# ducha-aiki/mods

Measured on AMD Instinct MI355X. Metric: image-pairs/sec (1024x768, HessAff+RootSIFT over the affine view ladder, MFMA FGINN match, LO-RANSAC H), higher is better.
Workload: dtype f32 (detect/describe) + u8 on the int8 matrix cores (distance matrix)

## Files before the change

include/modsx.h:

```cpp
#ifndef MODSX_H
#define MODSX_H
#include <stdint.h>
#ifdef __cplusplus
extern "C" {
#endif

#define MODSX_VERSION 100

typedef enum modsx_status {
  MODSX_OK = 0,
  MODSX_ERR_ARG = -1,
  MODSX_ERR_DEVICE = -2,
  MODSX_ERR_NOMEM = -3,
  MODSX_ERR_INTERNAL = -4,
  MODSX_ERR_CAPACITY = -5,
  MODSX_ERR_TIMEOUT = -6
} modsx_status;

enum { MODSX_FIXED_TH = 0, MODSX_RELATIVE_TH = 1, MODSX_FIXED_REG_NUMBER = 2, MODSX_RELATIVE_REG_NUMBER = 3,
       MODSX_NOT_LESS_THAN_REGIONS = 4 };
enum { MODSX_DET_HESSIAN = 0, MODSX_DET_DOG = 1, MODSX_DET_HARRIS = 2, MODSX_DET_MSER = 3 };
enum { MODSX_DESC_SIFT = 0, MODSX_DESC_ROOT_SIFT = 1, MODSX_DESC_HALF_SIFT = 2, MODSX_DESC_HALF_ROOT_SIFT = 3 };
#define MODSX_MAX_DESC 4
enum { MODSX_HESSIAN_DARK = 0, MODSX_HESSIAN_BRIGHT = 1, MODSX_HESSIAN_SADDLE = 2 };
// ... 118 lines not shown
int modsx_resize_half(modsx_ctx *ctx, const modsx_image *img, float *out, int *orows, int *ocols);

int modsx_response(modsx_ctx *ctx, const modsx_image *img, int detector_type, float norm, float *out);

int modsx_detect_affine_regions(const modsx_keypoint *kps, int n, int img_id, int det_type, modsx_region *out);

void modsx_default_mser_params(modsx_mser_params *p);
int modsx_detect_msers(modsx_ctx *ctx, const modsx_image *img, const modsx_mser_params *par, double tilt, double zoom,
                       modsx_keypoint **out);
int modsx_detect_msers_u8(const unsigned char *gray, int rows, int cols, const modsx_mser_params *par, double tilt,
                          double zoom, modsx_keypoint **out);

int modsx_detect_orientation(modsx_ctx *ctx, const modsx_image *img, const modsx_region *in, int n, double mrSize,
                             int patchSize, int doHalfSIFT, int maxAngNum, double th, int addUpRight,
                             modsx_region **out);

int modsx_reproject_regions(modsx_region *regs, int n, const double *H, int orig_w, int orig_h);
int modsx_reproject_regions_touch_boundary(modsx_region *regs, int n, const double *H, int orig_w, int orig_h, double mrSize);

int modsx_describe_regions(modsx_ctx *ctx, const modsx_image *img, const modsx_region *regs, int n, double mrSize,
                           int patchSize, int fast_extraction, int photoNorm, int desc_type, double maxBinValue,
                           float *desc);

int modsx_match_fginn(modsx_ctx *ctx, const float *desc1, int n1, const float *desc2, int n2, const double *pos2,
                      double ratio, double contradDist, int nn, modsx_tentative **out);

int modsx_duplicate_filtering(const double *pts, const double *key, int T, double r, int do_sort, int *order,
                              unsigned char *keep);

int modsx_ransac_h(const double *u, int len, double th, double conf, int max_sam, double *H, unsigned char *inl,
                   int *data_out, int oriented_constraint, int doSymCheck, unsigned seed, double *score_J);

int modsx_loransac_h(const double *pts, const double *laf1, const double *laf2, int T, double err_threshold,
                     double confidence, int max_samples, int localOptimization, double HLAFCoef, int doSymmCheck,
                     unsigned seed, double *H, double *Hraw, unsigned char *inl, unsigned char *keep,
                     int *data_out);

int modsx_ransac_h_errtype(const double *u, int len, double th, double conf, int max_sam, double *H, unsigned char *inl,
                           int *data_out, int oriented_constraint, int doSymCheck, int error_type, unsigned seed,
                           double *score_J);
int modsx_loransac_h_errtype(const double *pts, const double *laf1, const double *laf2, int T, double err_threshold,
                             double confidence, int max_samples, int localOptimization, double HLAFCoef, int doSymmCheck,
                             int error_type, unsigned seed, double *H, double *Hraw, unsigned char *inl,
                             unsigned char *keep, int *data_out);

int modsx_ransac_f(const double *u, int len, double th, double conf, int max_sam, int do_lo, unsigned inl_limit,
                   int error_type, int doSymCheck, unsigned seed, double *F, unsigned char *inl, int *data_out);

int modsx_loransac_f(const double *pts, const double *laf1, const double *laf2, int T, double err_threshold,
                     double confidence, int max_samples, int localOptimization, double LAFCoef, int doSymmCheck,
                     int error_type, unsigned seed, double *F, unsigned char *inl, unsigned char *keep, int *data_out);
int modsx_verify_device_stats(long *out, int reset);
int modsx_verify_device_timing(long *out, int reset);

int modsx_match_pair(modsx_ctx *ctx, const modsx_image *img1, const modsx_image *img2,
                     const modsx_pair_params *par, modsx_pair_result *res);
void modsx_pair_result_release(modsx_pair_result *res);

int modsx_match_pairs(modsx_ctx *const *ctxs, int n_ctx, const modsx_image *const *imgs1,
                      const modsx_image *const *imgs2, int n_pairs, const modsx_pair_params *par,
                      modsx_pair_result *results);

int modsx_match_pairs_views(modsx_ctx *const *ctxs, int n_ctx, const modsx_image *const *imgs1,
                            const modsx_image *const *imgs2, int n_pairs, const modsx_view *views, int n_views,
                            const modsx_pair_params *par, modsx_pair_result *results);

int modsx_last_batch_verify(double *sum_ms, int *pairs, int *threads);
int modsx_last_match_geometry(int *qs, int *fat, int *S, int *tiles_per_split, int *ntiles_ub);
int modsx_describe_counters(modsx_ctx *ctx, long *out, int n);
int modsx_debug_orientation_counts(unsigned long long *launched, unsigned long long *skipped, int reset);
int modsx_debug_reproject_certain_drop(const modsx_region *regs, int n, const double *H, int orig_w, int orig_h, double boxk,
                                       unsigned char *drop);
int modsx_debug_describe_plan(const modsx_region *regs, const int *counts, int nimages, double mr_size, int fast_extraction,
                              unsigned long long arena_floats, long *counters, int n, long *cuts, int cap_cuts, int *n_cuts);
int modsx_debug_baumberg_geometry(int n, int W, int variant, int chunk, int *geometry);
int modsx_debug_baumberg_geometry_ctx(modsx_ctx *ctx, int n, int W, int variant, int chunk, int *geometry);
int modsx_debug_baumberg_variant(int W);
int modsx_debug_baumberg(modsx_ctx *ctx, const modsx_image *const *planes, int nplanes, const int *plane_of, const float *xyspd,
                         int n, const modsx_hessaff_params *par, int variant, int chunk, float *u, int *ok, int *iters,
                         int *geometry, int *handed_out);
int modsx_debug_check_borders(const float *tuples, int n, unsigned char *touch);
int modsx_debug_describe_lanes(int P, long *counts);
int modsx_debug_describe_lane_map(int rows, int nc, int *rule, int *map, int cap);
int modsx_last_timings(modsx_ctx *ctx, double *ms6);

int modsx_set_vs_pars(const double *scale_set, int ns, const double *tilt_set, int nt, double phi_base,
                      double InitSigma, int doBlur, modsx_view *par, int cap, modsx_view *prev, int *nprev,
                      int cap_prev);

modsx_image *modsx_synth_view(modsx_ctx *ctx, const modsx_image *gray, const modsx_view *view, double *H9,
                              int *is_identity);

int modsx_detect_describe_views(modsx_ctx *ctx, const modsx_image *img, const modsx_view *views, int nviews,
                                const modsx_pair_params *par, int view_begin, int view_step, modsx_region **regs,
                                float **desc, void *dev_desc_u8, long dev_cap, int *view_counts);

int modsx_match_fginn_device(modsx_ctx *ctx, const void *dev_desc1_u8, int n1, const void *dev_desc2_u8, int n2,
                             const double *pos2, double ratio, double contradDist, int nn, modsx_tentative **out);

#define MODSX_DB_MAX_ROWS 16777216L
typedef struct modsx_db modsx_db;
modsx_db *modsx_db_create(modsx_ctx *ctx, const void *rows, long n, int dtype);
void modsx_db_free(modsx_ctx *ctx, modsx_db *db);
long modsx_db_rows(const modsx_db *db);
int modsx_db_nearest(modsx_ctx *ctx, const modsx_db *db, const float *desc, int n, float *dmin);
int modsx_match_fginn_db(modsx_ctx *ctx, const float *desc1, int n1, const float *desc2, int n2, const double *pos2,
                         double ratio, double contradDist, int nn, const modsx_db *db, modsx_tentative **out, double **d2byDB);
int modsx_match_fginn_db_device(modsx_ctx *ctx, const void *dev_desc1_u8, int n1, const void *dev_desc2_u8, int n2,
                                const double *pos2, double ratio, double contradDist, int nn, const modsx_db *db,
                                modsx_tentative **out, double **d2byDB);
int modsx_set_fginn_db(modsx_ctx *ctx, const modsx_db *db);

#define MODSX_HAMMING_MAX_BYTES 64
int modsx_match_hamming(modsx_ctx *ctx, const void *desc1, int n1, const void *desc2, int n2, int nbytes, int dtype,
                        double distanceThreshold, modsx_tentative **out);
int modsx_match_hamming_device(modsx_ctx *ctx, const void *dev_desc1_u8, int n1, const void *dev_desc2_u8, int n2, int nbytes,
                               double distanceThreshold, modsx_tentative **out);
int modsx_hamming_tentatives(const int *nn2, int n1, double distanceThreshold, modsx_tentative **out);
int modsx_debug_match_hamming(modsx_ctx *ctx, const void *dev_desc1_u8, int n1, const void *dev_desc2_u8, int n2, int nbytes,
                              int splits, int *nn2, int *geometry);
int modsx_debug_hamming_geometry(int n1, int n2, int nbytes, int splits, int *geometry);
int modsx_match_regions_hamming(modsx_ctx *ctx, const modsx_region *regs1, const void *desc1, int n1,
                                const modsx_region *regs2, const void *desc2, int n2, int nbytes, int dtype,
                                double distanceThreshold, const modsx_pair_params *par, modsx_pair_result *res);

int modsx_match_pair_views(modsx_ctx *ctx, const modsx_image *img1, const modsx_image *img2,
                           const modsx_view *views, int nviews, const modsx_pair_params *par,
                           modsx_pair_result *res);

typedef struct modsx_ladder_step {
  const modsx_view *views;
  int nviews;
  double match_ratio;
  int detector;
  int n_desc;
  int desc_types[MODSX_MAX_DESC];
  double desc_ratios[MODSX_MAX_DESC];
} modsx_ladder_step;
int modsx_match_ladder(modsx_ctx *ctx, const modsx_image *img1, const modsx_image *img2,
                       const modsx_ladder_step *steps, int nsteps, int min_matches, const modsx_pair_params *par,
                       modsx_pair_result *res, int *steps_done);

typedef struct modsx_rep modsx_rep;
modsx_rep *modsx_rep_create(modsx_ctx *ctx);
void modsx_rep_free(modsx_ctx *ctx, modsx_rep *rep);
int modsx_rep_add_views(modsx_ctx *ctx, modsx_rep *rep, const modsx_image *img, const modsx_ladder_step *step,
                        const modsx_pair_params *par);
int modsx_rep_append(modsx_ctx *ctx, modsx_rep *rep, int detector, int desc_type, const modsx_region *regs, const void *desc, int dtype,
                     int n);
int modsx_rep_class(modsx_ctx *ctx, const modsx_rep *rep, int detector, int desc_type, modsx_region **regs, unsigned char **desc_u8);
int modsx_rep_match_fginn(modsx_ctx *ctx, const modsx_rep *rep1, const modsx_rep *rep2, int detector, int desc_type, double ratio,
                          double contradDist, int nn, modsx_tentative **out);
typedef struct { int detector, desc_type; double ratio; } modsx_rep_class_sel;
int modsx_match_reps(modsx_ctx *const *ctxs, int n_ctx, const modsx_rep *rep1, const modsx_rep *const *reps2, int n,
                     const modsx_rep_class_sel *classes, int n_classes, const modsx_pair_params *par, modsx_pair_result *results);
int modsx_match_one_to_many(modsx_ctx *const *ctxs, int n_ctx, const modsx_image *img1, const modsx_image *const *imgs2, int n,
                            const modsx_ladder_step *steps, int nsteps, int min_matches, const modsx_pair_params *par,
                            modsx_pair_result *results, int *steps_done);

typedef struct modsx_comm modsx_comm;
int modsx_comm_unique_id(void *id128);
int modsx_comm_loopback_id(void *id128, int world);
modsx_comm *modsx_comm_create(modsx_ctx *ctx, const void *id128, int rank, int world);
void modsx_comm_destroy(modsx_comm *comm);
int modsx_comm_set_lanes(modsx_comm *comm, int nlanes);
int modsx_comm_attach(modsx_comm *comm, modsx_ctx *ctx, int lane);
// ... 55 lines not shown
```

mods_amd/__init__.py:

```python
import ctypes as C
import os
import subprocess

import numpy as np

_HERE = os.path.dirname(os.path.abspath(__file__))
LIB_PATH = os.environ.get("MODSX_LIB", os.path.join(_HERE, "libmodsx.so"))

KEYPOINT = np.dtype([("x", "f8"), ("y", "f8"), ("a11", "f8"), ("a12", "f8"), ("a21", "f8"), ("a22", "f8"),
                     ("s", "f8"), ("response", "f8"), ("octave_number", "i4"), ("pyramid_scale", "f8"),
                     ("sub_type", "i4")], align=True)
REGION = np.dtype([("img_id", "i4"), ("img_reproj_id", "i4"), ("id", "i4"), ("parent_id", "i4"), ("type", "i4"),
                   ("det_kp", KEYPOINT), ("reproj_kp", KEYPOINT)], align=True)
SSKP = np.dtype([("octave", "i4"), ("level", "i4"), ("r0", "i4"), ("c0", "i4"), ("r", "i4"), ("c", "i4"),
                 ("type", "i4"), ("pad", "i4"), ("b0", "f4"), ("b1", "f4"), ("b2", "f4"), ("val", "f4"),
                 ("x", "f4"), ("y", "f4"), ("s", "f4"), ("pixelDistance", "f4")], align=True)
TENT = np.dtype([("q", "i4"), ("t0", "i4"), ("tj", "i4"), ("t1", "i4"), ("d1", "f8"), ("d2", "f8"),
                 ("d2by2ndcl", "f8"), ("ratio", "f8")], align=True)


class HessAffParams(C.Structure):
    _fields_ = [("threshold", C.c_float), ("mode", C.c_int), ("reg_number", C.c_int),
                ("rel_threshold", C.c_float), ("rel_reg_number", C.c_float), ("numberOfScales", C.c_int),
                ("initialSigma", C.c_float), ("edgeEigenValueRatio", C.c_double), ("border", C.c_int),
                ("maxIterations", C.c_int), ("convergenceThreshold", C.c_float), ("smmWindowSize", C.c_int),
                ("affInitialSigma", C.c_float), ("doBaumberg", C.c_int), ("detectorType", C.c_int)]


class MserParams(C.Structure):
    _fields_ = [("min_size", C.c_int), ("max_area", C.c_double), ("min_margin", C.c_double), ("relative", C.c_int),
                ("mode", C.c_int), ("reg_number", C.c_int), ("rel_threshold", C.c_float), ("rel_reg_number", C.c_float)]


class PairParams(C.Structure):
    _fields_ = [("det", HessAffParams),
                ("ori_mrSize", C.c_double), ("ori_patchSize", C.c_int), ("ori_maxAngles", C.c_int),
                ("ori_threshold", C.c_double),
                ("desc_mrSize", C.c_double), ("desc_patchSize", C.c_int), ("desc_photoNorm", C.c_int),
                ("desc_type", C.c_int), ("desc_maxBinValue", C.c_double),
                ("match_ratio", C.c_double), ("contradDist", C.c_double), ("nn", C.c_int),
                ("duplicateDist", C.c_double),
                ("err_threshold", C.c_double), ("confidence", C.c_double), ("max_samples", C.c_int),
                ("localOptimization", C.c_int), ("HLAFCoef", C.c_double), ("doSymmCheck", C.c_int),
                ("ransac_seed", C.c_uint), ("useF", C.c_int), ("LAFCoef", C.c_double), ("errorType", C.c_int),
                ("detector", C.c_int), ("mser", MserParams),
                ("n_desc", C.c_int), ("desc_types", C.c_int * 4), ("desc_ratios", C.c_double * 4)]


class View(C.Structure):
    _fields_ = [("zoom", C.c_double), ("tilt", C.c_double), ("phi", C.c_double), ("InitSigma", C.c_double),
                ("doBlur", C.c_int)]


def make_view(tilt=1.0, phi=0.0, zoom=1.0, init_sigma=0.5, do_blur=1):
    v = View()
    v.zoom, v.tilt, v.phi, v.InitSigma, v.doBlur = zoom, tilt, phi, init_sigma, do_blur
    return v


def _view_array(views):
    arr = (View * len(views))()
    for i, v in enumerate(views):
        arr[i].zoom, arr[i].tilt, arr[i].phi, arr[i].InitSigma, arr[i].doBlur = v.zoom, v.tilt, v.phi, v.InitSigma, v.doBlur
    return arr


class LadderStep(C.Structure):
    _fields_ = [("views", C.c_void_p), ("nviews", C.c_int), ("match_ratio", C.c_double), ("detector", C.c_int),
                ("n_desc", C.c_int), ("desc_types", C.c_int * 4), ("desc_ratios", C.c_double * 4)]


class PairResult(C.Structure):
    _fields_ = [("n_regions1", C.c_int), ("n_regions2", C.c_int), ("n_tentatives", C.c_int), ("n_unique", C.c_int),
                ("n_ransac_inliers", C.c_int), ("n_verified", C.c_int), ("ransac_samples", C.c_int),
                ("ransac_lo", C.c_int), ("H", C.c_double * 9), ("tentatives", C.c_void_p),
                ("ransac_inlier", C.c_void_p), ("verified", C.c_void_p)]


class RepClassSel(C.Structure):
    _fields_ = [("detector", C.c_int), ("desc_type", C.c_int), ("ratio", C.c_double)]


EXPORTS = ["modsx_version", "modsx_last_error", "modsx_free", "modsx_create", "modsx_destroy", "modsx_synchronize",
           "modsx_default_hessaff_params", "modsx_default_pair_params", "modsx_image_upload", "modsx_image_update",
           "modsx_image_wrap_device", "modsx_image_free", "modsx_image_download", "modsx_detect_affine_keypoints",
           "modsx_detect_scalespace", "modsx_octave_levels", "modsx_gaussian_blur", "modsx_resize_half", "modsx_response",
           "modsx_detect_affine_regions", "modsx_detect_orientation", "modsx_reproject_regions", "modsx_reproject_regions_touch_boundary",
           "modsx_describe_regions", "modsx_match_fginn", "modsx_duplicate_filtering", "modsx_ransac_h",
           "modsx_loransac_h", "modsx_ransac_h_errtype", "modsx_loransac_h_errtype", "modsx_ransac_f", "modsx_loransac_f", "modsx_match_pair", "modsx_match_pairs", "modsx_match_pairs_views", "modsx_pair_result_release",
           "modsx_set_vs_pars", "modsx_synth_view", "modsx_detect_describe_views", "modsx_match_fginn_device",
           "modsx_match_pair_views", "modsx_match_ladder", "modsx_save_regions", "modsx_load_regions", "modsx_default_mser_params", "modsx_detect_msers", "modsx_detect_msers_u8", "modsx_last_timings", "modsx_profile",
           "modsx_kernel_stats", "modsx_last_batch_verify", "modsx_last_match_geometry", "modsx_describe_counters", "modsx_comm_unique_id", "modsx_comm_create", "modsx_comm_destroy", "modsx_comm_info",
           "modsx_view_block_order", "modsx_detect_describe_views_sharded", "modsx_match_fginn_sharded",
           "modsx_match_pair_views_sharded", "modsx_match_pairs_views_sharded", "modsx_match_ladder_sharded", "modsx_comm_loopback_id", "modsx_comm_set_lanes",
           "modsx_comm_attach", "modsx_comm_lane_done", "modsx_comm_reset_lanes", "modsx_comm_set_timeout", "modsx_comm_stats",
           "modsx_shard_block_bytes", "modsx_shard_block_pack", "modsx_shard_blocks_unpack", "modsx_shard_device_pack",
           "modsx_shard_device_unpack", "modsx_verify_device_stats", "modsx_verify_device_timing", "modsx_comm_set_exchange",
           "modsx_shard_owner_plan", "modsx_db_create", "modsx_db_free", "modsx_db_rows", "modsx_db_nearest",
           "modsx_match_fginn_db", "modsx_match_fginn_db_device", "modsx_set_fginn_db",
           "modsx_debug_orientation_counts", "modsx_debug_reproject_certain_drop", "modsx_debug_describe_plan",
           "modsx_debug_baumberg_geometry", "modsx_debug_baumberg_geometry_ctx", "modsx_debug_baumberg_variant",
           "modsx_debug_baumberg", "modsx_debug_check_borders", "modsx_debug_describe_lanes", "modsx_debug_describe_lane_map",
           "modsx_rep_create", "modsx_rep_free", "modsx_rep_add_views", "modsx_rep_append", "modsx_rep_class",
           "modsx_rep_match_fginn", "modsx_match_reps", "modsx_match_one_to_many",
           "modsx_match_hamming", "modsx_match_hamming_device", "modsx_hamming_tentatives", "modsx_debug_match_hamming",
           "modsx_match_regions_hamming", "modsx_debug_hamming_geometry"]
EXPORTS_DEGENSAC = ["exp_ransacHcustom", "exp_ransacFcustom", "HDs", "HDsi", "HDsidx", "HDsSym", "HDsiSym", "HDsSymidx",
                    "HDsSymMax", "HDsiSymMax", "HDsSymidxMax", "FDs", "FDsSym", "exFDs", "exFDsSym",
                    "modsx_ransac_set_seed"]

SHARD_ROW_REGION, SHARD_ROW_KP = 0, 1
EXCHANGE_ALL_GATHER, EXCHANGE_OWNER = 0, 1
DESCRIBE_COUNTERS = ("calls", "chunks", "max_chunks", "chunks_mid_image", "chunks_later_image", "jobs", "direct_jobs", "fused_windows",
                     "lds_row_tiles", "lds_col_tiles", "sample_tiles", "global_row_tiles", "global_col_tiles", "clamped_windows")
KP_FIELDS = ("x", "y", "a11", "a12", "a21", "a22", "s")
KERNEL_CLASSES = ["blur_hess", "hessian", "resize", "nms_localize", "baumberg", "orientation", "patch_sample",
                  "blur_rows", "describe", "match_fginn", "gray", "warp_affine", "view_blur", "blur_cols", "match_sweep1", "match_db"]


def build(force=False):
    src = os.path.join(_HERE, "csrc")
    srcs = [os.path.join(src, f) for f in os.listdir(src) if f.endswith((".hip", ".cpp", ".hpp"))]
    srcs.append(os.path.join(_HERE, "..", "include", "modsx.h"))
    stale = (not os.path.exists(LIB_PATH)) or any(os.path.getmtime(s) > os.path.getmtime(LIB_PATH) for s in srcs)
    if force or stale:
        subprocess.check_call(["make", "-C", src, "-j8"], stdout=subprocess.DEVNULL)
    return LIB_PATH


_lib = None


def lib():
    global _lib
    if _lib is None:
        if not os.path.exists(LIB_PATH):
            raise RuntimeError("libmodsx.so is not built; run __graft_entry__.build() (needs hipcc)")
        L = C.CDLL(LIB_PATH)
        L.modsx_last_error.restype = C.c_char_p
        L.modsx_create.restype = C.c_void_p
        L.modsx_create.argtypes = [C.c_int]
        L.modsx_comm_create.restype = C.c_void_p
        L.modsx_comm_create.argtypes = [C.c_void_p, C.c_void_p, C.c_int, C.c_int]
        L.modsx_comm_destroy.argtypes = [C.c_void_p]
        L.modsx_comm_info.argtypes = [C.c_void_p] + [C.c_void_p] * 5
        L.modsx_comm_loopback_id.argtypes = [C.c_void_p, C.c_int]
        L.modsx_comm_set_lanes.argtypes = [C.c_void_p, C.c_int]
        L.modsx_comm_attach.argtypes = [C.c_void_p, C.c_void_p, C.c_int]
        L.modsx_comm_lane_done.argtypes = [C.c_void_p, C.c_int]
        L.modsx_comm_reset_lanes.argtypes = [C.c_void_p]
        L.modsx_comm_set_timeout.argtypes = [C.c_void_p, C.c_int]
        L.modsx_comm_stats.argtypes = [C.c_void_p, C.c_void_p, C.c_int]
        L.modsx_destroy.argtypes = [C.c_void_p]
        L.modsx_free.argtypes = [C.c_void_p]
        L.modsx_image_upload.restype = C.c_void_p
        L.modsx_image_upload.argtypes = [C.c_void_p, C.c_void_p, C.c_int, C.c_int, C.c_int, C.c_int]
        L.modsx_image_update.argtypes = [C.c_void_p, C.c_void_p, C.c_void_p, C.c_int, C.c_int, C.c_int, C.c_int]
        L.modsx_debug_last_batch_verify_each.argtypes = [C.c_void_p, C.c_int]
        L.modsx_image_wrap_device.restype = C.c_void_p
        L.modsx_image_wrap_device.argtypes = [C.c_void_p, C.c_void_p, C.c_int, C.c_int]
        L.modsx_image_free.argtypes = [C.c_void_p, C.c_void_p]
        L.modsx_db_create.restype = C.c_void_p
        L.modsx_db_create.argtypes = [C.c_void_p, C.c_void_p, C.c_long, C.c_int]
        L.modsx_db_free.restype = None
        L.modsx_db_free.argtypes = [C.c_void_p, C.c_void_p]
        L.modsx_db_rows.restype = C.c_long
        L.modsx_db_rows.argtypes = [C.c_void_p]
        L.modsx_db_nearest.argtypes = [C.c_void_p, C.c_void_p, C.c_void_p, C.c_int, C.c_void_p]
        L.modsx_set_fginn_db.argtypes = [C.c_void_p, C.c_void_p]
        L.modsx_debug_reproject_certain_drop.argtypes = [C.c_void_p, C.c_int, C.c_void_p, C.c_int, C.c_int, C.c_double, C.c_void_p]
        L.modsx_describe_counters.argtypes = [C.c_void_p, C.c_void_p, C.c_int]
        L.modsx_debug_orientation_counts.argtypes = [C.c_void_p, C.c_void_p, C.c_int]
        L.modsx_debug_describe_plan.argtypes = [C.c_void_p, C.c_void_p, C.c_int, C.c_double, C.c_int, C.c_ulonglong, C.c_void_p, C.c_int,
                                                C.c_void_p, C.c_int, C.c_void_p]
        L.modsx_debug_baumberg_geometry.argtypes = [C.c_int, C.c_int, C.c_int, C.c_int, C.c_void_p]
        L.modsx_debug_baumberg.argtypes = [C.c_void_p, C.c_void_p, C.c_int, C.c_void_p, C.c_void_p, C.c_int, C.c_void_p, C.c_int, C.c_int,
                                           C.c_void_p, C.c_void_p, C.c_void_p, C.c_void_p, C.c_void_p]
        L.modsx_debug_baumberg_variant.argtypes = [C.c_int]
        L.modsx_debug_baumberg_geometry_ctx.argtypes = [C.c_void_p, C.c_int, C.c_int, C.c_int, C.c_int, C.c_void_p]
        L.modsx_debug_check_borders.argtypes = [C.c_void_p, C.c_int, C.c_void_p]
        L.modsx_debug_describe_lanes.argtypes = [C.c_int, C.c_void_p]
        L.modsx_debug_describe_lane_map.argtypes = [C.c_int, C.c_int, C.c_void_p, C.c_void_p, C.c_int]
        L.modsx_rep_create.restype = C.c_void_p
        L.modsx_rep_create.argtypes = [C.c_void_p]
        L.modsx_rep_free.restype = None
        L.modsx_rep_free.argtypes = [C.c_void_p, C.c_void_p]
        L.modsx_rep_add_views.argtypes = [C.c_void_p, C.c_void_p, C.c_void_p, C.c_void_p, C.c_void_p]
        L.modsx_rep_append.argtypes = [C.c_void_p, C.c_void_p, C.c_int, C.c_int, C.c_void_p, C.c_void_p, C.c_int, C.c_int]
        L.modsx_rep_class.argtypes = [C.c_void_p, C.c_void_p, C.c_int, C.c_int, C.c_void_p, C.c_void_p]
        L.modsx_rep_match_fginn.argtypes = [C.c_void_p, C.c_void_p, C.c_void_p, C.c_int, C.c_int, C.c_double, C.c_double, C.c_int,
                                            C.c_void_p]
        L.modsx_match_reps.argtypes = [C.c_void_p, C.c_int, C.c_void_p, C.c_void_p, C.c_int, C.c_void_p, C.c_int, C.c_void_p,
                                       C.c_void_p]
        L.modsx_match_one_to_many.argtypes = [C.c_void_p, C.c_int, C.c_void_p, C.c_void_p, C.c_int, C.c_void_p, C.c_int, C.c_int,
                                              C.c_void_p, C.c_void_p, C.c_void_p]
        L.modsx_match_hamming.argtypes = [C.c_void_p, C.c_void_p, C.c_int, C.c_void_p, C.c_int, C.c_int, C.c_int, C.c_double, C.c_void_p]
        L.modsx_match_hamming_device.argtypes = [C.c_void_p, C.c_void_p, C.c_int, C.c_void_p, C.c_int, C.c_int, C.c_double, C.c_void_p]
        L.modsx_hamming_tentatives.argtypes = [C.c_void_p, C.c_int, C.c_double, C.c_void_p]
        L.modsx_debug_match_hamming.argtypes = [C.c_void_p, C.c_void_p, C.c_int, C.c_void_p, C.c_int, C.c_int, C.c_int, C.c_void_p,
                                                C.c_void_p]
        L.modsx_debug_hamming_last_ms.argtypes = [C.c_void_p, C.c_void_p]
        L.modsx_match_regions_hamming.argtypes = [C.c_void_p, C.c_void_p, C.c_void_p, C.c_int, C.c_void_p, C.c_void_p, C.c_int, C.c_int,
                                                  C.c_int, C.c_double, C.c_void_p, C.c_void_p]
        L.modsx_synth_view.restype = C.c_void_p
        L.modsx_synth_view.argtypes = [C.c_void_p, C.c_void_p, C.c_void_p, C.c_void_p, C.c_void_p]
        _lib = L
    return _lib


def _err():
    return lib().modsx_last_error().decode()


def _p(a):
    return a.ctypes.data_as(C.c_void_p)


def _check(rc, what):
    if rc < 0:
        raise RuntimeError("%s failed (%d): %s" % (what, rc, _err()))
    return rc


def default_hessaff_params(**kw):
    p = HessAffParams()
    lib().modsx_default_hessaff_params(C.byref(p))
    for k, v in kw.items():
        setattr(p, k, v)
    return p


def default_mser_params(**kw):
    p = MserParams()
    lib().modsx_default_mser_params(C.byref(p))
    for k, v in kw.items():
        setattr(p, k, v)
    return p


def detect_msers_u8(gray, params=None, tilt=1.0, zoom=1.0):
    params = params or default_mser_params()
    g = np.ascontiguousarray(gray, np.uint8)
    out = C.c_void_p()
    n = _check(lib().modsx_detect_msers_u8(_p(g), g.shape[0], g.shape[1], C.byref(params), C.c_double(tilt),
                                           C.c_double(zoom), C.byref(out)), "detect_msers_u8")
    return _take(out, n, KEYPOINT)


def default_pair_params(**kw):
    p = PairParams()
    lib().modsx_default_pair_params(C.byref(p))
    descs = kw.pop("descs", None)
    if descs is not None:
        _set_descs(p, descs)
    for k, v in kw.items():
        if hasattr(p.det, k) and not hasattr(p, k):
            setattr(p.det, k, v)
        else:
            setattr(p, k, v)
    return p


def _set_descs(obj, descs):
    obj.n_desc = len(descs)
    for i, (t, r) in enumerate(descs):
# ... 280 lines not shown
        h = lib().modsx_image_wrap_device(self._c(), C.c_void_p(dev_ptr), rows, cols)
        if not h:
            raise RuntimeError("modsx_image_wrap_device failed: " + _err())
        return Image(self, h, rows, cols)

    def synchronize(self):
        _check(lib().modsx_synchronize(self._c()), "synchronize")

    def gaussian_blur(self, img, sigma):
        out = np.empty((img.rows, img.cols), np.float32)
        _check(lib().modsx_gaussian_blur(self._c(), C.c_void_p(img.h), C.c_float(sigma), _p(out)), "gaussian_blur")
        return out

    def response(self, img, detector_type, norm):
        out = np.zeros((img.rows, img.cols), np.float32)
        _check(lib().modsx_response(self._c(), C.c_void_p(img.h), int(detector_type), C.c_float(norm), _p(out)), "response")
        return out

    def resize_half(self, img):
        r, c = C.c_int(), C.c_int()
        _check(lib().modsx_resize_half(self._c(), C.c_void_p(img.h), None, C.byref(r), C.byref(c)), "resize_half")
        out = np.empty((r.value, c.value), np.float32)
        _check(lib().modsx_resize_half(self._c(), C.c_void_p(img.h), _p(out), C.byref(r), C.byref(c)), "resize_half")
        return out

    def octave_levels(self, img, params):
        L = params.numberOfScales + 2
        blurs = np.empty((L, img.rows, img.cols), np.float32)
        resps = np.empty((L, img.rows, img.cols), np.float32)
        _check(lib().modsx_octave_levels(self._c(), C.c_void_p(img.h), C.byref(params), _p(blurs), _p(resps)),
               "octave_levels")
        return blurs, resps

    def detect_scalespace(self, img, params):
        out = C.c_void_p()
        n = _check(lib().modsx_detect_scalespace(self._c(), C.c_void_p(img.h), C.byref(params), C.byref(out)),
                   "detect_scalespace")
        return _take(out, n, SSKP)

    def detect_affine_keypoints(self, img, params, tilt=1.0, zoom=1.0):
        out = C.c_void_p()
        n = _check(lib().modsx_detect_affine_keypoints(self._c(), C.c_void_p(img.h), C.byref(params),
                                                       C.c_double(tilt), C.c_double(zoom), C.byref(out)),
                   "detect_affine_keypoints")
        return _take(out, n, KEYPOINT)

    def debug_baumberg(self, planes, plane_of, xyspd, params, variant=0, chunk=0):
        plane_of = np.ascontiguousarray(plane_of, np.int32)
        xyspd = np.ascontiguousarray(xyspd, np.float32).reshape(-1, 4)
        n = len(plane_of)
        assert len(xyspd) == n
        ptrs = (C.c_void_p * max(1, len(planes)))(*[im.h for im in planes])
        u = np.zeros((max(n, 1), 4), np.float32)
        ok, iters = np.zeros(max(n, 1), np.int32), np.zeros(max(n, 1), np.int32)
        geo = np.zeros(4, np.int32)
        handed = C.c_int(0)
        _check(lib().modsx_debug_baumberg(self._c(), ptrs, len(planes), _p(plane_of), _p(xyspd), n, C.byref(params), int(variant),
                                          int(chunk), _p(u), _p(ok), _p(iters), _p(geo), C.byref(handed)), "debug_baumberg")
        return dict(u=u[:n], ok=ok[:n], iters=iters[:n], geometry=dict(zip(BAUMBERG_GEOMETRY, (int(x) for x in geo))),
                    handed_out=handed.value)

    def baumberg_geometry(self, n, W=19, variant=0, chunk=0):
        geo = np.zeros(4, np.int32)
        _check(lib().modsx_debug_baumberg_geometry_ctx(self._c(), int(n), int(W), int(variant), int(chunk), _p(geo)), "baumberg_geometry")
        return dict(zip(BAUMBERG_GEOMETRY, (int(x) for x in geo)))

    def detect_orientation(self, img, regs, mr_size=1.0, patch_size=41, half=0, max_ang=1, th=0.8, upright=0):
        regs = np.ascontiguousarray(regs, REGION)
        out = C.c_void_p()
        n = _check(lib().modsx_detect_orientation(self._c(), C.c_void_p(img.h), _p(regs), len(regs),
                                                  C.c_double(mr_size), patch_size, half, max_ang, C.c_double(th),
                                                  upright, C.byref(out)), "detect_orientation")
        return _take(out, n, REGION)

    def describe_regions(self, img, regs, mr_size=5.1962, patch_size=41, fast=0, photo_norm=1, desc_type=1,
                         max_bin=0.2):
        regs = np.ascontiguousarray(regs, REGION)
        desc = np.zeros((len(regs), 128), np.float32)
        _check(lib().modsx_describe_regions(self._c(), C.c_void_p(img.h), _p(regs), len(regs), C.c_double(mr_size),
                                            patch_size, fast, photo_norm, desc_type, C.c_double(max_bin), _p(desc)),
               "describe_regions")
        return desc

    def describe_counters(self):
        v = (C.c_long * len(DESCRIBE_COUNTERS))()
        n = _check(lib().modsx_describe_counters(self._c(), v, len(DESCRIBE_COUNTERS)), "describe_counters")
        assert n == len(DESCRIBE_COUNTERS), n
        return dict(zip(DESCRIBE_COUNTERS, (int(x) for x in v)))

    def match_fginn(self, d1, d2, pos2, ratio=0.8, contrad_dist=30.0, nn=50):
        d1 = np.ascontiguousarray(d1, np.float32)
        d2 = np.ascontiguousarray(d2, np.float32)
        pos2 = np.ascontiguousarray(pos2, np.float64)
        out = C.c_void_p()
        n = _check(lib().modsx_match_fginn(self._c(), _p(d1), len(d1), _p(d2), len(d2), _p(pos2), C.c_double(ratio),
                                           C.c_double(contrad_dist), nn, C.byref(out)), "match_fginn")
        return _take(out, n, TENT)

    def db_create(self, rows):
        a = np.ascontiguousarray(rows)
        if a.dtype != np.uint8:
            a = np.ascontiguousarray(a, np.float32)
        if a.ndim != 2 or a.shape[1] != 128:
            raise ValueError("db_create: an [n][128] array is expected")
        h = lib().modsx_db_create(self._c(), _p(a), a.shape[0], 0 if a.dtype == np.uint8 else 1)
        if not h:
            raise RuntimeError("modsx_db_create failed: " + _err())
        return Db(self, h)

    def db_nearest(self, db, desc):
        d = np.ascontiguousarray(desc, np.float32)
        out = np.empty(len(d), np.float32)
        _check(lib().modsx_db_nearest(self._c(), C.c_void_p(db.h), _p(d), len(d), _p(out)), "db_nearest")
        return out

    def match_fginn_db(self, d1, d2, pos2, db, ratio=0.8, contrad_dist=30.0, nn=50):
        d1 = np.ascontiguousarray(d1, np.float32)
        d2 = np.ascontiguousarray(d2, np.float32)
        pos2 = np.ascontiguousarray(pos2, np.float64)
        out, dd = C.c_void_p(), C.c_void_p()
        n = _check(lib().modsx_match_fginn_db(self._c(), _p(d1), len(d1), _p(d2), len(d2), _p(pos2), C.c_double(ratio),
                                              C.c_double(contrad_dist), nn, C.c_void_p(db.h if db is not None else None),
                                              C.byref(out), C.byref(dd)), "match_fginn_db")
        return _take(out, n, TENT), _take(dd, n, np.dtype("f8"))

    def match_fginn_db_device(self, d1_ptr, n1, d2_ptr, n2, pos2, db, ratio=0.8, contrad_dist=30.0, nn=50):
        pos2 = np.ascontiguousarray(pos2, np.float64)
        out, dd = C.c_void_p(), C.c_void_p()
        n = _check(lib().modsx_match_fginn_db_device(self._c(), C.c_void_p(d1_ptr), int(n1), C.c_void_p(d2_ptr), int(n2),
                                                     _p(pos2), C.c_double(ratio), C.c_double(contrad_dist), nn,
                                                     C.c_void_p(db.h), C.byref(out), C.byref(dd)), "match_fginn_db_device")
        return _take(out, n, TENT), _take(dd, n, np.dtype("f8"))

    def set_fginn_db(self, db):
        _check(lib().modsx_set_fginn_db(self._c(), C.c_void_p(db.h) if db is not None else None), "set_fginn_db")

    def synth_view(self, img, view):
        H = np.zeros(9)
        ident = C.c_int(0)
        h = lib().modsx_synth_view(self._c(), C.c_void_p(img.h), C.byref(view), _p(H), C.byref(ident))
        if not h:
            raise RuntimeError("modsx_synth_view failed: " + _err())
        rows, cols = C.c_int(), C.c_int()
        out = Image(self, h, 0, 0)
        out.rows, out.cols = _image_dims(h)
        return out, H.reshape(3, 3), bool(ident.value)

    def detect_describe_views(self, img, views, params, view_begin=0, view_step=1, want_desc=True, dev_desc=None,
                              dev_cap=0, want_counts=False):
        arr = _view_array(views)
        regs = C.c_void_p()
        desc = C.c_void_p()
        counts = (C.c_int * len(views))()
        n = _check(lib().modsx_detect_describe_views(self._c(), C.c_void_p(img.h), arr, len(views), C.byref(params),
                                                     int(view_begin), int(view_step), C.byref(regs),
                                                     C.byref(desc) if want_desc else None,
                                                     C.c_void_p(dev_desc) if dev_desc else None, C.c_long(dev_cap),
                                                     counts),
                   "detect_describe_views")
        r = _take(regs, n, REGION)
        d = None
        if want_desc:
            d = _take(desc, n * 128, np.dtype("f4")).reshape(n, 128) if n else np.zeros((0, 128), np.float32)
        if want_counts:
            return r, d, np.array(list(counts), np.int64)
        return r, d
# ... 183 lines not shown
    return out[:n]


def last_batch_verify():
    ms, n, t = C.c_double(), C.c_int(), C.c_int()
    lib().modsx_last_batch_verify(C.byref(ms), C.byref(n), C.byref(t))
    return ms.value, n.value, t.value


def last_match_geometry():
    v = [C.c_int() for _ in range(5)]
    lib().modsx_last_match_geometry(*[C.byref(x) for x in v])
    return dict(zip(("qs", "fat", "S", "tiles_per_split", "ntiles_ub"), (x.value for x in v)))


HAMMING_GEOMETRY = ("tile", "splits", "workgroups", "W")


def _hamming_rows(d1, d2):
    d1, d2 = np.asarray(d1), np.asarray(d2)
    dt = np.uint8 if d1.dtype == np.uint8 and d2.dtype == np.uint8 else np.float32
    d1, d2 = np.ascontiguousarray(d1, dt), np.ascontiguousarray(d2, dt)
    if d1.ndim != 2 or d2.ndim != 2 or d1.shape[1] != d2.shape[1]:
        raise ValueError("hamming: two [n][nbytes] arrays of one width are expected")
    return d1, d2, d1.shape[1], 0 if dt == np.uint8 else 1


def hamming_geometry(n1, n2, nbytes, splits=0):
    geo = np.zeros(4, np.int32)
    _check(lib().modsx_debug_hamming_geometry(int(n1), int(n2), int(nbytes), int(splits), _p(geo)), "hamming_geometry")
    return dict(zip(HAMMING_GEOMETRY, (int(x) for x in geo)))


def hamming_tentatives(nn2, distance_threshold):
    nn2 = np.ascontiguousarray(nn2, np.int32).reshape(-1, 4)
    out = C.c_void_p()
    n = _check(lib().modsx_hamming_tentatives(_p(nn2), len(nn2), C.c_double(distance_threshold), C.byref(out)), "hamming_tentatives")
    return _take(out, n, TENT)


BAUMBERG_GEOMETRY = ("kernel", "chunk", "nchunks", "grid")


def baumberg_geometry(n, W=19, variant=0, chunk=0):
    geo = np.zeros(4, np.int32)
    _check(lib().modsx_debug_baumberg_geometry(int(n), int(W), int(variant), int(chunk), _p(geo)), "baumberg_geometry")
    return dict(zip(BAUMBERG_GEOMETRY, (int(x) for x in geo)))


def baumberg_production_variant(W=19):
    return int(lib().modsx_debug_baumberg_variant(int(W)))


def check_borders(tuples):
    t = np.ascontiguousarray(tuples, np.float32).reshape(-1, 9)
    out = np.zeros(max(1, len(t)), np.uint8)
    _check(lib().modsx_debug_check_borders(_p(t), len(t), _p(out)), "check_borders")
    return out[:len(t)].astype(bool)


DESCRIBE_LANE_PHASES = ("sample", "rows", "cols_fused", "cols")


def describe_lanes(P):
    k = np.zeros(16, np.int64)
    _check(lib().modsx_debug_describe_lanes(int(P), _p(k)), "describe_lanes")
    out = dict(zip(("ksize", "NC", "rows0", "ro1"), (int(x) for x in k[:4])))
    for q, name in enumerate(DESCRIBE_LANE_PHASES):
        out[name] = tuple(int(x) for x in k[4 + 3 * q:7 + 3 * q])
    return out


def describe_lane_map(rows, nc=0):
    rule = np.zeros(5, np.int32)
    m = np.zeros((max(1, int(rows) * int(nc)), 3), np.int32)
    n = lib().modsx_debug_describe_lane_map(int(rows), int(nc), _p(rule), _p(m), len(m))
    if n < 0:
        _check(n, "describe_lane_map")
    out = dict(zip(("cols", "stride", "park_words", "magic", "slots"), (int(x) for x in rule)))
    out["map"] = m[:n]
    return out


def orientation_counts(reset=False):
    a, b = C.c_ulonglong(), C.c_ulonglong()
    lib().modsx_debug_orientation_counts(C.byref(a), C.byref(b), int(reset))
    return a.value, b.value


def reproject_certain_drop(regs, H, w, h, boxk=2 * 3.0 * 3.0 ** 0.5):
    regs = np.ascontiguousarray(regs, REGION)
    H = np.ascontiguousarray(H, np.float64).reshape(9)
    drop = np.zeros(max(1, len(regs)), np.uint8)
    _check(lib().modsx_debug_reproject_certain_drop(_p(regs), len(regs), _p(H), int(w), int(h), C.c_double(boxk), _p(drop)),
           "reproject_certain_drop")
    return drop[:len(regs)].astype(bool)


DEFAULT_ARENA_FLOATS = 192 << 18


def describe_plan(regs, mr_size, fast=0, arena_floats=DEFAULT_ARENA_FLOATS, max_cuts=4096):
    lists = [regs] if isinstance(regs, np.ndarray) else list(regs)
    counts = np.array([len(r) for r in lists], np.int32)
    flat = np.ascontiguousarray(np.concatenate([np.asarray(r).view(REGION) for r in lists]) if lists else np.zeros(0, REGION), REGION)
    cnt = (C.c_long * len(DESCRIBE_COUNTERS))()
    cuts = (C.c_long * max(1, max_cuts))()
    ncuts = C.c_int(0)
    rc = lib().modsx_debug_describe_plan(_p(flat), _p(counts), len(lists), C.c_double(mr_size), int(fast), int(arena_floats), cnt,
                                         len(DESCRIBE_COUNTERS), cuts, max_cuts, C.byref(ncuts))
    assert ncuts.value <= max_cuts, "describe_plan: %d cuts, room for %d" % (ncuts.value, max_cuts)
    return dict(rc=rc, error=_err() if rc else "", counters=dict(zip(DESCRIBE_COUNTERS, (int(x) for x in cnt))),
                cuts=[int(cuts[i]) for i in range(ncuts.value)])


def view_block_order(counts):
    counts = np.ascontiguousarray(counts, np.int32)
    world, nviews = counts.shape
    total = int(counts.sum())
    src = np.zeros(max(1, total), np.int32)
    mr = C.c_int(0)
    n = _check(lib().modsx_view_block_order(_p(counts), world, nviews, _p(src), len(src), C.byref(mr)), "view_block_order")
    return src[:n].copy(), mr.value


def shard_owner_plan(item_counts, nviews, world, rank, image_owner):
    cnt = np.ascontiguousarray(item_counts, np.int32)
    own = np.ascontiguousarray(image_owner, np.int32)
    nimg = len(own)
    assert len(cnt) == nimg * nviews
    cap = max(1, len(cnt), nimg * world)
    sends, recvs, jobs = (np.zeros((cap, 4), np.int32) for _ in range(3))
    n = (C.c_long * 5)()
    L = lib()
    L.modsx_shard_owner_plan.argtypes = [C.c_void_p, C.c_int, C.c_int, C.c_int, C.c_int, C.c_void_p, C.c_void_p, C.c_void_p, C.c_void_p, C.c_int, C.c_void_p]
    _check(L.modsx_shard_owner_plan(_p(cnt), nimg, nviews, world, rank, _p(own), _p(sends), _p(recvs), _p(jobs), cap, n), "shard_owner_plan")
    return {"sends": sends[:n[0]].copy(), "recvs": recvs[:n[1]].copy(), "jobs": jobs[:n[2]].copy(), "recv_rows": int(n[3]), "list_rows": int(n[4])}


def _ptr_array(arrs):
    return (C.c_void_p * len(arrs))(*[a.ctypes.data for a in arrs])


def shard_region_bytes(row_format):
    return REGION.itemsize if row_format == SHARD_ROW_REGION else 56


def shard_kp_rows(regs):
    k = np.asarray(regs)["reproj_kp"]
    return np.stack([k[f] for f in KP_FIELDS], 1).astype(np.float64) if len(k) else np.zeros((0, 7))


def shard_block_bytes(items, block_rows, ndesc=1, row_format=SHARD_ROW_REGION):
    L = lib()
    L.modsx_shard_block_bytes.restype = C.c_long
    return int(L.modsx_shard_block_bytes(int(items), int(block_rows), int(ndesc), int(row_format)))


def shard_block_pack(regs, descs, counts, block_rows, rc_local=0, row_format=SHARD_ROW_REGION):
    L = lib()
    L.modsx_shard_block_pack.restype = C.c_long
    regs = np.ascontiguousarray(regs, REGION)
    descs = [np.ascontiguousarray(d, np.uint8) for d in descs]
    counts = np.ascontiguousarray(counts, np.int32)
    out = np.zeros(shard_block_bytes(len(counts), block_rows, len(descs), row_format), np.uint8)
    n = _check(L.modsx_shard_block_pack(_p(regs), _ptr_array(descs), len(descs), len(regs), _p(counts), len(counts), int(rc_local),
# ... 114 lines not shown
```

mods_amd/csrc/capi.hip:

```cpp
#include <math.h>
#include <malloc.h>
#include <algorithm>
#include <atomic>
#include <chrono>
#include <mutex>
#include <thread>
#include <condition_variable>
#include <deque>
#include "engine_api.hpp"
#include "describe_plan.hpp"
#include "describe_lanes.hpp"

using namespace mx;

#define NEED(c)                                             \
  do {                                                      \
    if (!(c)) { mx::set_error("null argument: " #c); return MODSX_ERR_ARG; } \
  } while (0)

template <typename T>
static T *to_malloc(const std::vector<T> &v) {
  T *p = (T *)malloc(sizeof(T) * (v.size() ? v.size() : 1));
  if (p && !v.empty()) memcpy(p, v.data(), sizeof(T) * v.size());
  return p;
}

static std::atomic<long> g_verifyUs(0);
static std::atomic<int> g_verifyThreads(0), g_verifyPairs(0);
static std::mutex g_verifyEachMu;
static std::vector<int> g_verifyEachUs;
static void verify_timed(mx::VerifyTask &t, const modsx_pair_params &pp);
static std::atomic<long> g_cpuWorkerUs(0), g_cpuHelperUs(0);
static int verify_helpers(int nw) {
  static const int cap = getenv("MODSX_VERIFY_HELPERS") ? atoi(getenv("MODSX_VERIFY_HELPERS")) : 0;
  return cap > 0 ? (cap < nw ? cap : nw) : nw;
}
static long thread_cpu_us() { timespec t; clock_gettime(CLOCK_THREAD_CPUTIME_ID, &t); return t.tv_sec * 1000000L + t.tv_nsec / 1000; }
struct ThreadCpu { std::atomic<long> &acc; long t0; explicit ThreadCpu(std::atomic<long> &a) : acc(a), t0(thread_cpu_us()) {} ~ThreadCpu() { acc += thread_cpu_us() - t0; } };

extern "C" {

int modsx_version(void) { return MODSX_VERSION; }
const char *modsx_last_error(void) { return mx::last_error(); }
void modsx_free(void *p) { free(p); }

static void tune_host_allocator() {
#if defined(__GLIBC__)
  static std::once_flag once;
  std::call_once(once, [] {
    const char *e = getenv("MODSX_MALLOC_TUNE");
    if (!e || atoi(e) == 0) return;
    mallopt(M_MMAP_THRESHOLD, 1 << 30);
    mallopt(M_TRIM_THRESHOLD, 1 << 30);
    mallopt(M_TOP_PAD, 64 << 20);
  });
#endif
}

modsx_ctx *modsx_create(int device_id) {
  tune_host_allocator();
  return ctx_create(device_id);
}
void modsx_destroy(modsx_ctx *ctx) { ctx_destroy(ctx); }
int modsx_synchronize(modsx_ctx *ctx) {
  NEED(ctx);
  MX_HIP(hipStreamSynchronize(ctx->stream));
  return MODSX_OK;
}

void modsx_default_hessaff_params(modsx_hessaff_params *p) {
  p->threshold = 5.3333f;
  p->mode = MODSX_FIXED_TH;
  p->reg_number = 2000;
  p->rel_threshold = -1;
  p->rel_reg_number = -1;
  p->numberOfScales = 3;
  p->initialSigma = 1.6f;
  p->edgeEigenValueRatio = 10.0;
  p->border = 5;
  p->maxIterations = 16;
  p->convergenceThreshold = 0.05f;
  p->smmWindowSize = 19;
  p->affInitialSigma = 1.6f;
  p->doBaumberg = 1;
  p->detectorType = MODSX_DET_HESSIAN;
}

void modsx_default_mser_params(modsx_mser_params *p);
void modsx_default_pair_params(modsx_pair_params *p) {
  memset(p, 0, sizeof *p);
  modsx_default_hessaff_params(&p->det);
  p->ori_mrSize = 1.0; p->ori_patchSize = 41; p->ori_maxAngles = 1; p->ori_threshold = 0.8;
  p->desc_mrSize = 5.1962; p->desc_patchSize = 41; p->desc_photoNorm = 1; p->desc_type = MODSX_DESC_ROOT_SIFT;
  p->desc_maxBinValue = 0.2;
// ... 234 lines not shown
  int rc = detect_orientation_batch(ctx, imgs, 1, vin, mrSize, patchSize, doHalfSIFT, maxAngNum, th, addUpRight, vout);
  if (rc) return rc;
  *out = to_malloc(vout[0]);
  return (int)vout[0].size();
}

int modsx_reproject_regions(modsx_region *regs, int n, const double *H, int orig_w, int orig_h) {
  if (n < 0 || (n > 0 && !regs) || !H) { mx::set_error("modsx_reproject_regions: bad argument"); return MODSX_ERR_ARG; }
  return reproject_regions(regs, n, H, orig_w, orig_h);
}

int modsx_reproject_regions_touch_boundary(modsx_region *regs, int n, const double *H, int orig_w, int orig_h, double mrSize) {
  if (n < 0 || (n > 0 && !regs) || !H) { mx::set_error("modsx_reproject_regions_touch_boundary: bad argument"); return MODSX_ERR_ARG; }
  return reproject_regions_box(regs, n, H, orig_w, orig_h, mrSize);
}

int modsx_debug_reproject_certain_drop(const modsx_region *regs, int n, const double *H, int orig_w, int orig_h, double boxk,
                                       unsigned char *drop) {
  if (n < 0 || (n > 0 && (!regs || !drop)) || !H) { mx::set_error("modsx_debug_reproject_certain_drop: bad argument"); return MODSX_ERR_ARG; }
  reproject_certain_drop(regs, n, H, orig_w, orig_h, boxk, drop);
  return n;
}

int modsx_debug_orientation_counts(unsigned long long *launched, unsigned long long *skipped, int reset) {
  mx::orientation_counts(launched, skipped, reset != 0);
  return MODSX_OK;
}

int modsx_debug_baumberg_geometry(int n, int W, int variant, int chunk, int *geometry) {
  NEED(geometry);
  const mx::BaumGeo g = mx::baumberg_geometry(n, W, variant, chunk);
  geometry[0] = g.kernel; geometry[1] = g.chunk; geometry[2] = g.nchunks; geometry[3] = g.grid;
  if (g.kernel < 0) { mx::set_error("modsx_debug_baumberg_geometry: no kernel for this window size / variant / chunk"); return MODSX_ERR_ARG; }
  return MODSX_OK;
}

int modsx_debug_baumberg_geometry_ctx(modsx_ctx *ctx, int n, int W, int variant, int chunk, int *geometry) {
  NEED(ctx); NEED(geometry);
  hipSetDevice(ctx->dev);
  return debug_baumberg_geometry(ctx, n, W, variant, chunk, geometry);
}

int modsx_debug_baumberg_variant(int W) { return mx::baumberg_production_variant(W); }

int modsx_debug_describe_lanes(int P, long *counts) {
  NEED(counts);
  if (P < 3) { mx::set_error("modsx_debug_describe_lanes: no such window"); return MODSX_ERR_ARG; }
  mx::DescSizePlan sp;
  const int rc = mx::describe_size_plan(P, sp);
  if (rc) return rc;
  mx::LaneCount k[4] = {};
  const int NP = (sp.NC + 1) / 2;
  for (int r0 = 0; sp.rows0 > 0 && r0 < P; r0 += sp.rows0) {
    const int nr = std::min(sp.rows0, P - r0);
    mx::lanes_count_sampling(P, nr, mx::BF_T / 64, k[0]);
    mx::lanes_count_filter(nr * NP, k[1]);
  }
  if (sp.ro1 < 0) mx::lanes_count_filter(sp.NC * NP, k[2]);
  for (int ro0 = 0; sp.ro1 > 0 && ro0 < sp.NC; ro0 += sp.ro1) mx::lanes_count_filter(std::min(sp.ro1, sp.NC - ro0) * NP, k[3]);
  counts[0] = sp.ksize; counts[1] = sp.NC; counts[2] = sp.rows0; counts[3] = sp.ro1;
  for (int q = 0; q < 4; q++) { counts[4 + 3 * q] = k[q].useful; counts[5 + 3 * q] = k[q].issued; counts[6 + 3 * q] = k[q].issuedParent; }
  return MODSX_OK;
}

int modsx_debug_describe_lane_map(int rows, int nc, int *rule, int *map, int cap) {
  NEED(rule);
  if (rows < 1 || rows > 64) { mx::set_error("modsx_debug_describe_lane_map: a row pass has 1 .. 64 rows"); return MODSX_ERR_ARG; }
  constexpr mx::SrLaneTable T = mx::sr_lane_table();
  const int ncFull = mx::sr_table_cols(T.w[rows]), CP = mx::sr_stride(ncFull);
  rule[0] = ncFull; rule[1] = CP; rule[2] = mx::SR_PARK; rule[3] = 0; rule[4] = 0;
  if (nc == 0) return 0;
  if (nc < 0 || nc > ncFull || cap < 0 || (cap > 0 && !map)) { mx::set_error("modsx_debug_describe_lane_map: bad argument"); return MODSX_ERR_ARG; }
  const unsigned magic = mx::sr_table_magic(T.w[nc]);
  const int tot = rows * nc;
  rule[3] = (int)magic; rule[4] = mx::sr_slots(rows, nc);
  for (int e = 0; e < tot && e < cap; e++) {
    unsigned r, c;
    mx::sr_sample_rc((unsigned)e, nc, magic, r, c);
    map[3 * e] = (int)r; map[3 * e + 1] = (int)c; map[3 * e + 2] = (int)(r * (unsigned)CP + c);
  }
  return tot;
}

int modsx_debug_baumberg(modsx_ctx *ctx, const modsx_image *const *planes, int nplanes, const int *plane_of, const float *xyspd,
                         int n, const modsx_hessaff_params *par, int variant, int chunk, float *u, int *ok, int *iters,
                         int *geometry, int *handed_out) {
  NEED(ctx); NEED(par); NEED(geometry);
  if (n < 0 || nplanes < 0 || (nplanes > 0 && !planes) || (n > 0 && (!plane_of || !xyspd || !u || !ok || !iters))) {
    mx::set_error("modsx_debug_baumberg: bad argument"); return MODSX_ERR_ARG;
  }
  hipSetDevice(ctx->dev);
  return debug_baumberg(ctx, planes, nplanes, plane_of, xyspd, n, *par, variant, chunk, u, ok, iters, geometry, handed_out);
}

int modsx_debug_check_borders(const float *tuples, int n, unsigned char *touch) {
  if (n < 0 || (n > 0 && (!tuples || !touch))) { mx::set_error("modsx_debug_check_borders: bad argument"); return MODSX_ERR_ARG; }
  for (int i = 0; i < n; i++) {
    const float *t = tuples + 9 * (size_t)i;
    touch[i] = mx::check_borders((int)t[0], (int)t[1], t[2], t[3], t[4], t[5], t[6], t[7], (int)t[8], (int)t[8]) ? 1 : 0;
  }
  return n;
}

int modsx_describe_counters(modsx_ctx *ctx, long *out, int n) {
  NEED(ctx);
  if (n < 0 || (n > 0 && !out)) { mx::set_error("modsx_describe_counters: bad argument"); return MODSX_ERR_ARG; }
  long sum[mx::DC_N] = {0};
  for (const modsx_ctx *head : {(const modsx_ctx *)ctx, (const modsx_ctx *)ctx->peer})
    for (const modsx_ctx *c = head; c; c = c->half)
      for (int q = 0; q < mx::DC_N; q++)
        if (q == mx::DC_MAX_CHUNKS) sum[q] = std::max(sum[q], c->descCnt[q]); else sum[q] += c->descCnt[q];
  for (int q = 0; q < n && q < mx::DC_N; q++) out[q] = sum[q];
  return mx::DC_N;
}

int modsx_debug_describe_plan(const modsx_region *regs, const int *counts, int nimages, double mr_size, int fast_extraction,
                              unsigned long long arena_floats, long *counters, int n, long *cuts, int cap_cuts, int *n_cuts) {
  if (nimages < 0 || (nimages > 0 && !counts) || n < 0 || (n > 0 && !counters) || cap_cuts < 0 || (cap_cuts > 0 && !cuts) || !n_cuts) {
    mx::set_error("modsx_debug_describe_plan: bad argument"); return MODSX_ERR_ARG;
  }
  if (nimages > mx::MAXB) { mx::set_error("describe batch too large"); return MODSX_ERR_ARG; }
  std::vector<modsx_region> v[mx::MAXB];
  long first[mx::MAXB + 1] = {0};
  for (int i = 0; i < nimages; i++) {
    if (counts[i] < 0 || (counts[i] > 0 && !regs)) { mx::set_error("modsx_debug_describe_plan: bad argument"); return MODSX_ERR_ARG; }
    v[i].assign(regs + first[i], regs + first[i] + counts[i]);
    first[i + 1] = first[i] + counts[i];
  }
  mx::HostMark hm;
  mx::DescBatch batch;
  batch.regs = v; batch.n = nimages; batch.mrSize = mr_size; batch.fast = fast_extraction;
  mx::DescCursor cur = mx::describe_windows(batch);
  long cnt[mx::DC_N] = {0};
  int chunkNo = 0, rc = MODSX_OK;
  *n_cuts = 0;
  cnt[mx::DC_CALLS]++;
  for (; cur.img < nimages; chunkNo++) {
    mx::DescChunkPlan cp;
    if (chunkNo) { if (*n_cuts < cap_cuts) cuts[*n_cuts] = first[cur.img] + (long)cur.reg; (*n_cuts)++; }
    rc = mx::describe_plan_chunk(batch, cur, (size_t)arena_floats, cp, hm);
    for (int q = 0; q < mx::DC_N; q++) cnt[q] += cp.cnt[q];
    if (rc) break;
    cur = cp.next;
  }
  if (!rc) cnt[mx::DC_MAX_CHUNKS] = chunkNo;
  for (int q = 0; q < n && q < mx::DC_N; q++) counters[q] = cnt[q];
  return rc;
}

int modsx_describe_regions(modsx_ctx *ctx, const modsx_image *img, const modsx_region *regs, int n, double mrSize,
                           int patchSize, int fast_extraction, int photoNorm, int desc_type, double maxBinValue,
                           float *desc) {
  NEED(ctx); NEED(img);
  if (n < 0 || (n > 0 && (!regs || !desc))) { mx::set_error("modsx_describe_regions: bad argument"); return MODSX_ERR_ARG; }
  if (desc_type < MODSX_DESC_SIFT || desc_type > MODSX_DESC_HALF_ROOT_SIFT) { mx::set_error("descriptor type"); return MODSX_ERR_ARG; }
  hipSetDevice(ctx->dev);
  std::vector<modsx_region> v[1];
  v[0].assign(regs, regs + n);
  const modsx_image *imgs[1] = {img};
  float *hosts[1] = {desc};
  int rc = describe_batch(ctx, imgs, 1, v, mrSize, patchSize, fast_extraction, photoNorm, desc_type, maxBinValue, hosts,
                          nullptr, nullptr);
  if (rc) return rc;
  return n;
}

int modsx_match_fginn(modsx_ctx *ctx, const float *desc1, int n1, const float *desc2, int n2, const double *pos2,
                      double ratio, double contradDist, int nn, modsx_tentative **out) {
  NEED(ctx); NEED(out);
  if (n1 < 0 || n2 < 0 || (n1 > 0 && !desc1) || (n2 > 0 && (!desc2 || !pos2))) { mx::set_error("modsx_match_fginn: bad argument"); return MODSX_ERR_ARG; }
  hipSetDevice(ctx->dev);
  std::vector<modsx_tentative> t;
  int rc = match_host_desc(ctx, desc1, n1, desc2, n2, pos2, ratio, contradDist, nn, t);
  if (rc) return rc;
  *out = to_malloc(t);
  return (int)t.size();
}

int modsx_duplicate_filtering(const double *pts, const double *key, int T, double r, int do_sort, int *order,
                              unsigned char *keep) {
  if (T < 0 || (T > 0 && (!pts || !order || !keep))) { mx::set_error("modsx_duplicate_filtering: bad argument"); return MODSX_ERR_ARG; }
  return duplicate_filtering(pts, key, T, r, do_sort, order, keep);
}

int modsx_ransac_h(const double *u, int len, double th, double conf, int max_sam, double *H, unsigned char *inl,
                   int *data_out, int oriented_constraint, int doSymCheck, unsigned seed, double *score_J) {
  if (!u || !H || !inl || !data_out || len < 4) { mx::set_error("modsx_ransac_h: bad argument"); return MODSX_ERR_ARG; }
  return ransac_h(u, len, th, conf, max_sam, H, inl, data_out, oriented_constraint, doSymCheck, seed, score_J);
}

int modsx_ransac_h_errtype(const double *u, int len, double th, double conf, int max_sam, double *H, unsigned char *inl,
                           int *data_out, int oriented_constraint, int doSymCheck, int error_type, unsigned seed, double *score_J) {
  if (!u || !H || !inl || !data_out || len < 4 || error_type < 0 || error_type > 2) { mx::set_error("modsx_ransac_h_errtype: bad argument"); return MODSX_ERR_ARG; }
  return ransac_h(u, len, th, conf, max_sam, H, inl, data_out, oriented_constraint, doSymCheck, seed, score_J, error_type);
}

int modsx_ransac_f(const double *u, int len, double th, double conf, int max_sam, int do_lo, unsigned inl_limit,
                   int error_type, int doSymCheck, unsigned seed, double *F, unsigned char *inl, int *data_out) {
  if (!u || !F || !inl || !data_out || len < 8) { mx::set_error("modsx_ransac_f: bad argument"); return MODSX_ERR_ARG; }
  return ransac_f(u, len, th, conf, max_sam, F, inl, data_out, do_lo, inl_limit, error_type, doSymCheck, seed);
}

int modsx_loransac_f(const double *pts, const double *laf1, const double *laf2, int T, double err_threshold,
                     double confidence, int max_samples, int localOptimization, double LAFCoef, int doSymmCheck,
                     int error_type, unsigned seed, double *F, unsigned char *inl, unsigned char *keep, int *data_out) {
  if (!pts || !laf1 || !laf2 || !F || !inl || !keep || !data_out || T < 0) {
    mx::set_error("modsx_loransac_f: bad argument");
    return MODSX_ERR_ARG;
  }
  return loransac_f(pts, laf1, laf2, T, err_threshold, confidence, max_samples, localOptimization, LAFCoef, doSymmCheck,
                    error_type, seed, F, inl, keep, data_out);
}

int modsx_loransac_h(const double *pts, const double *laf1, const double *laf2, int T, double err_threshold,
                     double confidence, int max_samples, int localOptimization, double HLAFCoef, int doSymmCheck,
                     unsigned seed, double *H, double *Hraw, unsigned char *inl, unsigned char *keep, int *data_out) {
  if (T < 0 || !H || !Hraw || !data_out || (T > 0 && (!pts || !laf1 || !laf2 || !inl || !keep))) {
    mx::set_error("modsx_loransac_h: bad argument");
    return MODSX_ERR_ARG;
  }
  return loransac_h(pts, laf1, laf2, T, err_threshold, confidence, max_samples, localOptimization, HLAFCoef, doSymmCheck,
                    seed, H, Hraw, inl, keep, data_out);
}

int modsx_loransac_h_errtype(const double *pts, const double *laf1, const double *laf2, int T, double err_threshold,
                             double confidence, int max_samples, int localOptimization, double HLAFCoef, int doSymmCheck,
                             int error_type, unsigned seed, double *H, double *Hraw, unsigned char *inl, unsigned char *keep,
                             int *data_out) {
  if (T < 0 || !H || !Hraw || !data_out || (T > 0 && (!pts || !laf1 || !laf2 || !inl || !keep)) || error_type < 0 || error_type > 2) {
    mx::set_error("modsx_loransac_h_errtype: bad argument");
    return MODSX_ERR_ARG;
  }
  return loransac_h(pts, laf1, laf2, T, err_threshold, confidence, max_samples, localOptimization, HLAFCoef, doSymmCheck,
                    seed, H, Hraw, inl, keep, data_out, error_type);
}

static void verify_timed(mx::VerifyTask &t, const modsx_pair_params &pp) {
  const auto v0 = std::chrono::steady_clock::now();
  mx::verify_tentatives(t.l1, t.l2, t.tents, pp, t.res);
  const long us = std::chrono::duration_cast<std::chrono::microseconds>(std::chrono::steady_clock::now() - v0).count();
  g_verifyUs += us;
  g_verifyPairs++;
  std::lock_guard<std::mutex> lk(g_verifyEachMu);
  g_verifyEachUs.push_back((int)us);
}
struct DeviceGuard {
// ... 733 lines not shown
```

mods_amd/csrc/engine.hip:

```cpp
#include <atomic>
#include <math.h>
#include <stdio.h>
#include <algorithm>
#include <chrono>
#include <map>
#include <unordered_set>
#include <mutex>
#include <string>
#include "engine_api.hpp"
#include "describe_plan.hpp"

#ifdef MODSX_DUP_BUILD
namespace mx {
int dup_count(int cls) {
  static const long mask = getenv("MODSX_DUP") ? strtol(getenv("MODSX_DUP"), nullptr, 0) : 0;
  return 1 + (int)((mask >> cls) & 1);
}
}
#endif
namespace mx {

static thread_local std::string g_err;
void set_error(const std::string &s) { g_err = s; }
static std::atomic<int> g_busyContexts{0};
bool gpu_shared() { return g_busyContexts.load(std::memory_order_relaxed) > 1; }
CtxBusy::CtxBusy(modsx_ctx *ctx) : c(ctx) {
  if (c && c->busyDepth++ == 0) {
    g_busyContexts.fetch_add(1, std::memory_order_relaxed);
    const bool rt = host_wait_runtime() || !c->hFlag;
    if (rt && !c->waitRuntime) hipStreamSynchronize(c->stream);
    c->waitRuntime = rt;
  }
}
CtxBusy::~CtxBusy() { if (c && --c->busyDepth == 0) g_busyContexts.fetch_sub(1, std::memory_order_relaxed); }
const char *last_error() { return g_err.c_str(); }

bool DevBuf::ensure(size_t bytes) {
  if (bytes <= cap) return true;
  release();
  size_t want = bytes + bytes / 4 + 256;
  if (hipMalloc(&p, want) != hipSuccess) { p = nullptr; cap = 0; set_error("hipMalloc failed"); return false; }
  cap = want;
  return true;
}
void DevBuf::release() { if (p) hipFree(p); p = nullptr; cap = 0; }
bool PinBuf::ensure(size_t bytes) {
  if (bytes <= cap) return true;
  release();
  size_t want = bytes + bytes / 4 + 256;
  if (hipHostMalloc(&p, want, hipHostMallocDefault) != hipSuccess) { p = nullptr; cap = 0; set_error("hipHostMalloc failed"); return false; }
  cap = want;
  return true;
}
void PinBuf::release() { if (p) hipHostFree(p); p = nullptr; cap = 0; }

}
#include <sys/prctl.h>
#include <time.h>
namespace mx {
__global__ void k_flag(unsigned *flag, unsigned seq) {
  __threadfence_system();
  __hip_atomic_store(flag, seq, __ATOMIC_RELEASE, __HIP_MEMORY_SCOPE_SYSTEM);
}
template <bool HOST_SRC>
__global__ __launch_bounds__(256) void k_copy_pinned(uint4 *dst, const uint4 *src, size_t n16, int tail) {
  if (HOST_SRC) __builtin_amdgcn_fence(__ATOMIC_ACQUIRE, "");
  const size_t stride = (size_t)gridDim.x * 256;
  size_t i = (size_t)blockIdx.x * 256 + threadIdx.x;
  for (; i + 3 * stride < n16; i += 4 * stride) {
    const uint4 a = src[i], b = src[i + stride], c = src[i + 2 * stride], d = src[i + 3 * stride];
    dst[i] = a; dst[i + stride] = b; dst[i + 2 * stride] = c; dst[i + 3 * stride] = d;
  }
  for (; i < n16; i += stride) dst[i] = src[i];
  if (tail && blockIdx.x == 0 && threadIdx.x < (unsigned)tail)
    reinterpret_cast<unsigned char *>(dst + n16)[threadIdx.x] = reinterpret_cast<const unsigned char *>(src + n16)[threadIdx.x];
  if (!HOST_SRC) __builtin_amdgcn_fence(__ATOMIC_RELEASE, "");
}
}
#include <sys/resource.h>
namespace mx {
bool host_wait_runtime() {
  static const int forced = [] {
    const char *e = getenv("MODSX_HOST_WAIT");
    if (e && !strcmp(e, "runtime")) return 1;
    if (e && !strcmp(e, "flag")) return 0;
    if (e && !strcmp(e, "alternate")) return 2;
    return -1;
  }();
  if (forced == 2) { static std::atomic<unsigned> flip{0}; return (flip.fetch_add(1, std::memory_order_relaxed) & 1) != 0; }
  if (forced >= 0) return forced != 0;
  static const double allowance = (double)host_cpus_per_rank();
  static std::atomic<int> rt{allowance >= 8 ? 1 : 0};
  static std::atomic<long long> nextNs{0};
// ... 70 lines not shown

static size_t prof_take_slot(Profiler &p, int cls, double work) {
  if (p.used == p.evA.size()) {
    hipEvent_t a, b;
    hipEventCreate(&a); hipEventCreate(&b);
    p.evA.push_back(a); p.evB.push_back(b); p.cls.push_back(0);
  }
  const size_t slot = p.used++;
  p.cls[slot] = cls;
  p.work[cls] += work;
  p.launches[cls]++;
  return slot;
}
void prof_begin(modsx_ctx *c, int cls, double work, size_t *slot) {
  *slot = (size_t)-1;
  if (!c->prof.enabled) return;
  *slot = prof_take_slot(c->prof, cls, work);
  hipEventRecord(c->prof.evA[*slot], c->stream);
}
void prof_end(modsx_ctx *c, size_t slot) { if (slot != (size_t)-1) hipEventRecord(c->prof.evB[slot], c->stream); }
bool prof_reserve(modsx_ctx *c, int cls, double work, hipEvent_t *ev2) {
  if (!c->prof.enabled) return false;
  const size_t slot = prof_take_slot(c->prof, cls, work);
  ev2[0] = c->prof.evA[slot]; ev2[1] = c->prof.evB[slot];
  return true;
}
void prof_collect(modsx_ctx *c) {
  Profiler &p = c->prof;
  if (!p.enabled || !p.used) return;
  hipStreamSynchronize(c->stream);
  for (size_t i = 0; i < p.used; i++) {
    float ms = 0;
    if (hipEventElapsedTime(&ms, p.evA[i], p.evB[i]) == hipSuccess) p.ms[p.cls[i]] += ms;
  }
  p.used = 0;
}
void prof_reset(modsx_ctx *c, bool enable) {
  Profiler &p = c->prof;
  p.enabled = enable; p.used = 0;
  for (int i = 0; i < K_NCLASS; i++) { p.ms[i] = 0; p.work[i] = 0; p.launches[i] = 0; }
}

static int upload_tables(modsx_ctx *c) {
  const int PS = 41;
  std::vector<float> m(PS * PS);
  circular_gauss_mask(m.data(), PS, PS / 3.0f);
  {
    const int PSP = 44;
    std::vector<unsigned short> idx;
    std::vector<float> w;
    for (int r = 1; r < PS - 1; r++)
      for (int q = 1; q < PS - 1; q++)
        if (m[r * PS + q] > 0) { idx.push_back((unsigned short)(r * PSP + q)); w.push_back(m[r * PS + q]); }
    for (int r = 0; r < PS; r++)
      for (int q = 0; q < PS; q++)
        if ((r == 0 || q == 0 || r == PS - 1 || q == PS - 1) && m[r * PS + q] > 0) {
          set_error("orientation mask reaches the patch frame");
          return MODSX_ERR_ARG;
        }
    if ((int)idx.size() > ORI_NV) { set_error("orientation voting list exceeds ORI_NV"); return MODSX_ERR_ARG; }
    while ((int)idx.size() < ORI_NV) { idx.push_back((unsigned short)(PSP + 1)); w.push_back(0.f); }
    {
      constexpr int PER_L = ORI_NV / 64;
      std::vector<unsigned short> idx2(ORI_NV);
      std::vector<float> w2(ORI_NV);
      for (int l = 0; l < 64; l++)
        for (int q = 0; q < PER_L; q++) { idx2[l + 64 * q] = idx[PER_L * l + q]; w2[l + 64 * q] = w[PER_L * l + q]; }
      idx.swap(idx2); w.swap(w2);
    }
    MX_HIP(hipMalloc(&c->dOriMask, ORI_NV * 4));
    MX_HIP(hipMalloc(&c->dOriIdx, ORI_NV * 2));
    MX_HIP(hipMemcpy(c->dOriMask, w.data(), ORI_NV * 4, hipMemcpyHostToDevice));
    MX_HIP(hipMemcpy(c->dOriIdx, idx.data(), ORI_NV * 2, hipMemcpyHostToDevice));
  }
  MX_HIP(hipMalloc(&c->dSiftMask, PS * PS * 4));
  circular_gauss_mask(m.data(), PS, 0);
  MX_HIP(hipMemcpy(c->dSiftMask, m.data(), PS * PS * 4, hipMemcpyHostToDevice));
  {
    std::vector<unsigned short> idx;
    for (int i = 0; i < PS * PS; i++) if (m[i] > 0) idx.push_back((unsigned short)i);
    c->nSiftMask = (int)idx.size();
    MX_HIP(hipMalloc(&c->dSiftMaskIdx, idx.size() * 2));
    MX_HIP(hipMemcpy(c->dSiftMaskIdx, idx.data(), idx.size() * 2, hipMemcpyHostToDevice));
  }
  MX_HIP(hipMalloc(&c->dAtan, 256 * 8));
  MX_HIP(hipMemcpy(c->dAtan, atan_lut_host(), 256 * 8, hipMemcpyHostToDevice));
  {
    std::vector<unsigned char> obin(ATAN_CASES);
    std::vector<float> so(ATAN_CASES);
    const double *L = atan_lut_host();
    const float PIf = float(M_PI);
    const double TWO_PI = 6.28318530718;
    for (int e = 0; e < ATAN_CASES; e++) {
      const float ori = e < 2048 ? atan2lut_value(L, e >> 8, e & 255) : 0.f;
      obin[e] = (unsigned char)(int)(36 * (ori / PIf + 1.0f) / 2.0f);
      so[e] = (float)((double)8.0f * ((double)ori + TWO_PI) / TWO_PI);
    }
    MX_HIP(hipMalloc(&c->dOriBinTab, ATAN_CASES));
    MX_HIP(hipMemcpy(c->dOriBinTab, obin.data(), ATAN_CASES, hipMemcpyHostToDevice));
    MX_HIP(hipMalloc(&c->dSiftOTab, ATAN_CASES * 4));
    MX_HIP(hipMemcpy(c->dSiftOTab, so.data(), ATAN_CASES * 4, hipMemcpyHostToDevice));
  }
  int bins[2 * PS];
  double w[2 * PS];
  const int spatialBins = 4, orientationBins = 8;
  int halfSize = PS >> 1;
  float step = float(spatialBins + 1) / (2 * halfSize);
  for (int i = 0; i < PS; i++) {
    float x = step * i;
    int xi = (int)(x);
    int b0 = xi - 1, b1 = xi;
    double w1 = x - xi;
    double w0 = 1.0f - w1;
    if (b0 < 0) { b0 = 0; w0 = 0; }
    if (b0 >= spatialBins) { b0 = spatialBins - 1; w0 = 0; }
    if (b1 < 0) { b1 = 0; w1 = 0; }
    if (b1 >= spatialBins) { b1 = spatialBins - 1; w1 = 0; }
    bins[i] = b0 * orientationBins; bins[PS + i] = b1 * orientationBins;
    w[i] = w0; w[PS + i] = w1;
    if ((double)(float)w0 != w0 || (double)(float)w1 != w1) { set_error("SIFT spatial weights are not f32 values"); return MODSX_ERR_ARG; }
  }
  MX_HIP(hipMalloc(&c->dSiftBins, sizeof bins));
  MX_HIP(hipMemcpy(c->dSiftBins, bins, sizeof bins, hipMemcpyHostToDevice));
  MX_HIP(hipMalloc(&c->dSiftW, sizeof w));
  MX_HIP(hipMemcpy(c->dSiftW, w, sizeof w, hipMemcpyHostToDevice));
  return MODSX_OK;
}

modsx_ctx *ctx_create(int device_id) {
  int ndev = 0;
  if (hipGetDeviceCount(&ndev) != hipSuccess || ndev <= 0) {
    set_error("no HIP device visible: libmodsx needs an MI355X (gfx950); there is no CPU fallback");
    return nullptr;
  }
  if (device_id < 0 || device_id >= ndev) { set_error("device id out of range"); return nullptr; }
  if (hipSetDevice(device_id) != hipSuccess) { set_error("hipSetDevice failed"); return nullptr; }
  {
    static std::once_flag once[64];
    if (device_id < 64)
      std::call_once(once[device_id], [device_id] {
        const char *e = getenv("MODSX_SYNC");
        if (e && !strcmp(e, "spin")) return;
        const unsigned flag = (e && !strcmp(e, "yield")) ? hipDeviceScheduleYield : hipDeviceScheduleBlockingSync;
        if (hipSetDeviceFlags(flag) != hipSuccess) {
          (void)hipGetLastError();
          fprintf(stderr, "modsx: hipSetDeviceFlags(hipDeviceScheduleBlockingSync) failed on device %d; host threads will spin-wait\n", device_id);
        }
      });
  }
  modsx_ctx *c = new modsx_ctx();
  c->dev = device_id;
  if (hipStreamCreate(&c->stream) != hipSuccess) { set_error("hipStreamCreate failed"); delete c; return nullptr; }
  for (int i = 0; i < 2; i++) hipEventCreateWithFlags(&c->descEv[i], hipEventDisableTiming);
  if (hipHostMalloc((void **)&c->hFlag, 64, hipHostMallocDefault) != hipSuccess) { set_error("hipHostMalloc failed"); hipStreamDestroy(c->stream); delete c; return nullptr; }
  c->hFlag[0] = 0; c->flagSeq = 0;
  c->waitRuntime = host_wait_runtime();
  for (int i = 0; i < 6; i++) c->timings[i] = 0;
  if (upload_tables(c) != MODSX_OK) { delete c; return nullptr; }
  return c;
}

void ctx_destroy(modsx_ctx *c) {
  if (!c) return;
  ctx_worker_stop(c);
  if (c->peer) { ctx_destroy(c->peer); c->peer = nullptr; }
  if (c->half) { ctx_destroy(c->half); c->half = nullptr; }
  hipSetDevice(c->dev);
  hipStreamSynchronize(c->stream);
  for (int i = 0; i < MAXB; i++) c->pyr[i].store.release();
  DevBuf *bufs[] = {&c->nmsJobs, &c->cand, &c->counter, &c->affJobs, &c->affOut, &c->oriJobs, &c->oriOut, &c->descJobs, &c->tilePrefix,
                    &c->taps, &c->imgRefs, &c->scratchA, &c->scratchB, &c->descAllF[0], &c->descAllF[1], &c->descAllU8[0],
                    &c->descAllU8[1], &c->descAllU8b[0], &c->descAllU8b[1], &c->shardLocal, &c->pos2, &c->matchRows, &c->matchWork, &c->dbSel, &c->misc, &c->scratchC, &c->needTab, &c->coordTab, &c->tileJob, &c->blurTiles, &c->nmsQueue, &c->rowStarts, &c->viewTmp[0], &c->viewTmp[1], &c->viewTaps, &c->viewJobs};
  for (DevBuf *b : bufs) b->release();
  for (int i = 0; i < MAXB; i++) { c->descF[i].release(); c->descU8[i].release(); c->viewImg[i].release(); for (int k = 0; k < 3; k++) c->descU8x[k][i].release(); }
  for (int d = 0; d < 2; d++) for (int t = 0; t < 4; t++) for (int sd = 0; sd < 2; sd++) c->descCls[d][t][sd].release();
  for (int t = 0; t < 4; t++) c->halfDesc[t].release();
  c->candSort.release(); c->candOut.release();
  PinBuf *pins[] = {&c->hCand, &c->hAff, &c->hOri, &c->hDesc, &c->hMisc, &c->hNms, &c->hMatch, &c->hViewTaps, &c->hViewJobs, &c->hMser};
  for (PinBuf *b : pins) b->release();
  hipFree(c->dSmmMask); hipFree(c->dOriMask); hipFree(c->dOriIdx); hipFree(c->dSiftMask); hipFree(c->dSiftMaskIdx); hipFree(c->dAtan); hipFree(c->dOriBinTab); hipFree(c->dSiftOTab); hipFree(c->dSiftBins);
  hipFree(c->dSiftW);
  for (int i = 0; i < 2; i++) hipEventDestroy(c->descEv[i]);
  c->hDescB.release(); c->hRefs.release();
  hipStreamDestroy(c->stream);
  if (c->hFlag) hipHostFree(c->hFlag);
  delete c;
}

static const double K_SIGMA = 2 * 3.0 * sqrt(3.0);

void desc_class_order(const DescSet &ds, int *ord) {
  int m = 0;
  for (int type = 3; type >= 0; type--)
    for (int i = 0; i < ds.n; i++) if (ds.type[i] == type) ord[m++] = i;
}
int resolve_descs(const modsx_pair_params &pp, const modsx_ladder_step *st, DescSet &ds) {
  const int ns = st ? st->n_desc : 0;
  if (ns < 0 || ns > MODSX_MAX_DESC || pp.n_desc < 0 || pp.n_desc > MODSX_MAX_DESC) { set_error("n_desc must be 0..4"); return MODSX_ERR_ARG; }
  if (ns > 0) { ds.n = ns; for (int i = 0; i < ns; i++) { ds.type[i] = st->desc_types[i]; ds.ratio[i] = st->desc_ratios[i]; } }
  else if (pp.n_desc > 0) { ds.n = pp.n_desc; for (int i = 0; i < ds.n; i++) { ds.type[i] = pp.desc_types[i]; ds.ratio[i] = pp.desc_ratios[i]; } }
  else { ds.n = 1; ds.type[0] = pp.desc_type; ds.ratio[0] = st && st->match_ratio > 0 ? st->match_ratio : pp.match_ratio; }
  for (int i = 0; i < ds.n; i++) {
    if (ds.type[i] < 0 || ds.type[i] > 3) { set_error("descriptor type must be 0..3 (SIFT, RootSIFT, HalfSIFT, HalfRootSIFT)"); return MODSX_ERR_ARG; }
    for (int j = 0; j < i; j++) if (ds.type[j] == ds.type[i]) { set_error("a descriptor type is listed twice in one step"); return MODSX_ERR_ARG; }
  }
  return MODSX_OK;
}

static int upload_img_refs(modsx_ctx *c, const modsx_image *const *imgs, int n) {
  const bool fresh = !c->imgRefs.p;
  if (!c->imgRefs.ensure(MAXB * sizeof(ImgRef))) return MODSX_ERR_NOMEM;
  ImgRef refs[MAXB];
  memset(refs, 0, sizeof refs);
  for (int i = 0; i < n; i++) { refs[i].d = imgs[i]->d; refs[i].rows = imgs[i]->rows; refs[i].cols = imgs[i]->cols; }
  if (!fresh && memcmp(refs, c->imgRefsHost, sizeof refs) == 0) return MODSX_OK;
  if (!c->hRefs.ensure(sizeof refs)) return MODSX_ERR_NOMEM;
  memcpy(c->hRefs.p, refs, sizeof refs);
  MX_HIP(ctx_copy(c, c->imgRefs.p, c->hRefs.p, sizeof refs, hipMemcpyHostToDevice));
  memcpy(c->imgRefsHost, refs, sizeof refs);
  return MODSX_OK;
}

static double eye_test(const double *H) {
  return fabs(H[0] - 1.0) + fabs(H[1]) + fabs(H[2]) + fabs(H[3]) + fabs(H[4] - 1.0) + fabs(H[5]) + fabs(H[6]) + fabs(H[7]) +
         fabs(H[8] - 1.0);
}
static bool is_eye(const double *H) { return eye_test(H) < 0.01; }
static bool ori_prefilter_on() {
  static const bool on = !(getenv("MODSX_ORI_PREFILTER") && atoi(getenv("MODSX_ORI_PREFILTER")) == 0);
  return on;
}
static std::atomic<unsigned long long> g_oriLaunched{0}, g_oriSkipped{0};
void orientation_counts(unsigned long long *launched, unsigned long long *skipped, bool reset) {
  if (launched) *launched = reset ? g_oriLaunched.exchange(0) : g_oriLaunched.load();
  else if (reset) g_oriLaunched.store(0);
  if (skipped) *skipped = reset ? g_oriSkipped.exchange(0) : g_oriSkipped.load();
  else if (reset) g_oriSkipped.store(0);
}

int detect_orientation_batch(modsx_ctx *c, const modsx_image *const *imgs, int n, const std::vector<modsx_region> *in,
                             double mrSize, int patchSize, int doHalfSIFT, int maxAngNum, double th, int addUpRight,
                             std::vector<modsx_region> *out, const OriReproj *reproj) {
  if (patchSize != 41) { set_error("orientation patchSize must be 41"); return MODSX_ERR_ARG; }
  const bool prefilter = reproj && ori_prefilter_on();
  for (int i = 0; i < n; i++) out[i].clear();
  double mrScale = (double)mrSize;
  int patchImageSize = 2 * int(mrScale) + 1;
  double imageToPatchScale = double(patchImageSize) / (double)patchSize;
  HostMark hm;
  std::vector<OriJob> jobs;
  std::vector<char> passed[MAXB];
  std::vector<unsigned char> certain[MAXB];
  std::vector<OriJob> jobsOf[MAXB];
  host_parallel_light(n, [&](int i) {
    passed[i].assign(in[i].size(), 0);
    jobsOf[i].clear();
    jobsOf[i].reserve(in[i].size());
    const bool sameTest = prefilter && reproj[i].orig_w == imgs[i]->cols && reproj[i].orig_h == imgs[i]->rows && is_eye(reproj[i].H);
    if (prefilter && !sameTest) {
      certain[i].resize(in[i].size());
      reproject_certain_drop(in[i].data(), (int)in[i].size(), reproj[i].H, reproj[i].orig_w, reproj[i].orig_h, K_SIGMA, certain[i].data());
    }
    unsigned long long nSkipped = 0;
// ... 112 lines not shown
  double Hi[9];
  invert3(H, Hi);
  const double lim[2] = {(double)(float)(orig_w - 3), (double)(float)(orig_h - 3)};
  for (int i = 0; i < n; i++) {
    drop[i] = 0;
    const modsx_keypoint &k = regs[i].det_kp;
    double c[2] = {k.x, k.y};
    double m[2][2] = {{k.a11, k.a12}, {k.a21, k.a22}};
    double hi1[2] = {1.0, 1.0};
    if (!eye) {
      c[0] = (Hi[0] * k.x + Hi[1] * k.y + Hi[2]);
      c[1] = (Hi[3] * k.x + Hi[4] * k.y + Hi[5]);
      m[0][0] = (Hi[0] * k.a11 + Hi[1] * k.a21);
      m[0][1] = (Hi[0] * k.a12 + Hi[1] * k.a22);
      m[1][0] = (Hi[3] * k.a11 + Hi[4] * k.a21);
      m[1][1] = (Hi[3] * k.a12 + Hi[4] * k.a22);
      hi1[0] = fabs(Hi[0]) + fabs(Hi[1]);
      hi1[1] = fabs(Hi[3]) + fabs(Hi[4]);
    }
    const double box = boxk * k.s;
    const double a1 = fabs(k.a11) + fabs(k.a12) + fabs(k.a21) + fabs(k.a22);
    if (!std::isfinite(c[0]) || !std::isfinite(c[1]) || !std::isfinite(m[0][0] + m[0][1] + m[1][0] + m[1][1]) || !std::isfinite(a1) ||
        !std::isfinite(hi1[0] + hi1[1]) || !(fabs(box) < 2e9))
      continue;
    if (!(fabs(c[0]) + fabs(c[1]) + fabs(m[0][0]) + fabs(m[0][1]) + fabs(m[1][0]) + fabs(m[1][1]) < 1e25)) continue;
    if (!((c[0] < orig_w) && (c[1] < orig_h) && (c[0] > 0) && (c[1] > 0))) { drop[i] = 1; continue; }
    const double hw = fabs((double)(float)ceil((double)(float)(int)box / 2.0));
    for (int r = 0; r < 2; r++) {
      const double d = hw * sqrt(m[r][0] * m[r][0] + m[r][1] * m[r][1]);
      const double e64 = hw * 0x1p-50 * hi1[r] * a1;
      const double margin = 0x1p-17 * (fabs(c[r]) + 3.0 * d) + 32.0 * e64;
      if (!std::isfinite(d) || !std::isfinite(margin)) continue;
      if (c[r] - d < 1.0 - margin || c[r] + d > lim[r] + margin) drop[i] = 1;
    }
  }
}

static int launch_describe_chunk(modsx_ctx *c, const DescChunkPlan &cp, int slot, HostMark &hm, int photoNorm, const DescSet &ds,
                                 double maxBin, const DescOut &outs) {
  hipStream_t s = c->stream;
  const size_t nj = cp.jobs.size();
  const int nS = cp.pfxSample.back(), nR = cp.pfxRow.back(), nC = cp.pfxCol.back(), nRL = cp.pfxRowL.back(), nCL = cp.pfxColL.back();
  const DescBlobLayout L(cp);
  PinBuf &hblob = slot ? c->hDescB : c->hDesc;
  if (c->descEvPending[slot]) { MX_HIP(c->descByEvent[slot] ? hipEventSynchronize(c->descEv[slot]) : ctx_wait_mark(c, c->descMark[slot])); c->descEvPending[slot] = false; }
  if (!c->descJobs.ensure(L.blobB) || !hblob.ensure(L.blobB) ||
      !c->scratchA.ensure(std::max<size_t>(1, cp.arenaA) * 4) || !c->scratchB.ensure(std::max<size_t>(1, cp.arenaB) * 4) ||
      !c->scratchC.ensure(std::max<size_t>(1, cp.arenaC) * 4) || !c->rowStarts.ensure(std::max<size_t>(1, cp.rowStarts) * 8) ||
      !c->tileJob.ensure(((size_t)nS + nR + nC + 3) * 4))
    return MODSX_ERR_NOMEM;
  int *tjS = (int *)c->tileJob.p, *tjR = tjS + nS, *tjC = tjR + nR;
  if (!c->blurTiles.ensure(((size_t)nRL + nCL + 1) * sizeof(BlurTile))) return MODSX_ERR_NOMEM;
  BlurTile *btR = (BlurTile *)c->blurTiles.p, *btC = btR + nRL;
  char *hb = (char *)hblob.p, *db = (char *)c->descJobs.p;
  describe_fill_blob(cp, L, hb);
  hm.mark("desc tables + blob");
  MX_HIP(ctx_copy(c, db, hb, L.blobB, hipMemcpyHostToDevice));
  c->descByEvent[slot] = c->waitRuntime || !c->hFlag;
  if (c->descByEvent[slot]) MX_HIP(hipEventRecord(c->descEv[slot], s)); else c->descMark[slot] = ctx_mark(c);
  c->descEvPending[slot] = true;
  int *dPfxS = (int *)(db + L.pfx(0)), *dPfxR = (int *)(db + L.pfx(1)), *dPfxC = (int *)(db + L.pfx(2));
  int *dPfxRL = (int *)(db + L.pfx(3)), *dPfxCL = (int *)(db + L.pfx(4));
  float *dTaps = (float *)(db + L.oTaps), *dCoord = (float *)(db + L.oCoord);
  int *dNeed = (int *)(db + L.oNeed);
  const DescJob *dj = (const DescJob *)(db + L.oJobs);
  if (nS) launch_expand_tiles(s, dPfxS, (int)nj, tjS);
  if (nR) launch_expand_tiles(s, dPfxR, (int)nj, tjR);
  if (nC) launch_expand_tiles(s, dPfxC, (int)nj, tjC);
  if (nRL + nCL)
    launch_expand_blur_tiles(s, dj, dPfxRL, dPfxCL, (int)nj, dNeed, btR, btC, (float2 *)c->rowStarts.p);
  { ProfScope ps(c, K_PATCH_SAMPLE, (double)cp.windowFloats * 4);
    launch_sample_rows(s, dj, btR, nRL, (ImgRef *)c->imgRefs.p, dTaps, dNeed, (float *)c->scratchB.p,
                       (const float2 *)c->rowStarts.p, (float *)c->scratchC.p);
    launch_patch_sample(s, dj, dPfxS, tjS, nS, (ImgRef *)c->imgRefs.p, (float *)c->scratchA.p); }
  { ProfScope ps(c, K_BLUR_ROWS, 0.0);
    launch_patch_blur(s, dj, dPfxR, tjR, nR, dTaps, dNeed, (float *)c->scratchA.p,
                      (float *)c->scratchB.p, 0); }
  { ProfScope ps(c, K_BLUR_COLS, 0.0);
    launch_blur_cols(s, btC, nCL, dTaps, dNeed, (float *)c->scratchB.p, (float *)c->scratchC.p);
    launch_patch_blur(s, dj, dPfxC, tjC, nC, dTaps, dNeed, (float *)c->scratchB.p,
                      (float *)c->scratchC.p, 1); }
  ProfScope psd(c, K_DESCRIBE, (double)nj * 128 * ds.n);
  launch_describe(s, dj, (int)nj, (ImgRef *)c->imgRefs.p, (float *)c->scratchC.p, dNeed, dCoord,
                  c->dSiftMask, c->dSiftMaskIdx, c->nSiftMask, c->dSiftOTab,
                  c->dSiftBins, c->dSiftW, photoNorm, ds.packed(), ds.n, maxBin, outs);
  return MODSX_OK;
}

int describe_batch(modsx_ctx *c, const modsx_image *const *imgs, int n, const std::vector<modsx_region> *regs,
                   double mrSize, int patchSize, int fast, int photoNorm, int descType, double maxBin,
                   float *const *descHost, float *const *devF, uint8_t *const *devU8, const DescSet *ds,
                   uint8_t *const *const *devU8x) {
  if (patchSize != 41) { set_error("descriptor patchSize must be 41"); return MODSX_ERR_ARG; }
  DescSet one;
  if (!ds) { one.n = 1; one.type[0] = descType; ds = &one; }
  if (ds->n < 1 || ds->n > MODSX_MAX_DESC) { set_error("describe: 1..4 descriptor classes"); return MODSX_ERR_ARG; }
  if (n > MAXB) { set_error("describe batch too large"); return MODSX_ERR_ARG; }
  hipStream_t s = c->stream;
  int rc = upload_img_refs(c, imgs, n);
  if (rc) return rc;
  static const size_t arenaMB = getenv("MODSX_ARENA_MB") ? (size_t)atol(getenv("MODSX_ARENA_MB")) : 192;
  const size_t ARENA_FLOATS = std::max<size_t>(arenaMB, 16) << 18;
  DescOut outs;
  memset(&outs, 0, sizeof outs);
  for (int i = 0; i < n; i++) {
    const size_t nr = regs[i].size();
    float *outF = devF ? devF[i] : nullptr;
    uint8_t *outU8 = devU8 ? devU8[i] : nullptr;
    if (!outF) { if (!c->descF[i].ensure(std::max<size_t>(1, nr) * 128 * 4)) return MODSX_ERR_NOMEM; outF = (float *)c->descF[i].p; }
    if (!outU8) { if (!c->descU8[i].ensure(std::max<size_t>(1, nr) * 128)) return MODSX_ERR_NOMEM; outU8 = (uint8_t *)c->descU8[i].p; }
    outs.f[i] = outF; outs.u8[i] = outU8;
    for (int k = 1; k < ds->n; k++) {
      uint8_t *o = devU8x && devU8x[k - 1] ? devU8x[k - 1][i] : nullptr;
      if (!o) { if (!c->descU8x[k - 1][i].ensure(std::max<size_t>(1, nr) * 128)) return MODSX_ERR_NOMEM; o = (uint8_t *)c->descU8x[k - 1][i].p; }
      outs.u8x[k - 1][i] = o;
    }
  }
  HostMark hm;
  DescBatch batch;
  batch.regs = regs; batch.n = n; batch.mrSize = mrSize; batch.fast = fast;
  DescCursor cur = describe_windows(batch);
  int chunkNo = 0;
  c->descCnt[DC_CALLS]++;
  for (; cur.img < n; chunkNo++) {
    DescChunkPlan cp;
    const int prc = describe_plan_chunk(batch, cur, ARENA_FLOATS, cp, hm);
    for (int q = 0; q < DC_N; q++) c->descCnt[q] += cp.cnt[q];
    if (prc) return prc;
    rc = launch_describe_chunk(c, cp, chunkNo & 1, hm, photoNorm, *ds, maxBin, outs);
    if (rc) return rc;
    cur = cp.next;
  }
  c->descCnt[DC_MAX_CHUNKS] = std::max<long>(c->descCnt[DC_MAX_CHUNKS], chunkNo);
  hm.mark("desc launches");
  MX_HIP(ctx_sync(c));
  hm.mark("desc wait");
  c->descEvPending[0] = c->descEvPending[1] = false;
  if (descHost) {
    bool any = false;
    for (int i = 0; i < n; i++)
      if (descHost[i] && !regs[i].empty()) {
        MX_HIP(hipMemcpyAsync(descHost[i], outs.f[i], regs[i].size() * 128 * 4, hipMemcpyDeviceToHost, s));
        any = true;
      }
    if (any) MX_HIP(hipStreamSynchronize(s));
  }
  MX_HIP(hipGetLastError());
  return MODSX_OK;
}

void rows_to_tentatives(const MatchRow *rows, int n1, int nn, std::vector<modsx_tentative> &o, const int *ddb, double sqminratio,
                        std::vector<double> *d2byDB) {
  o.reserve(n1 / 4 + 16);
  if (d2byDB) d2byDB->clear();
  for (int q = 0; q < n1; q++) {
    const MatchRow &r = rows[q];
    if (r.t0 < 0 || r.tj < 0 || r.nbad != 0 || r.nless > nn - 2) continue;
    modsx_tentative t;
    t.q = q; t.t0 = r.t0; t.tj = r.tj;
    t.t1 = r.t1;
    t.d1 = r.d0; t.d2 = r.dj; t.d2by2ndcl = r.d1;
    double ratio = r.d0 / r.dj;
    if (ddb) {
      const float dDB = (float)ddb[q];
      if (sqminratio < 1.0) {
        const double ratioDB = r.d0 / dDB;
        if (ratio < ratioDB) ratio = ratioDB;
// ... 418 lines not shown
```

mods_amd/csrc/engine.hpp:

```cpp
#pragma once
#include <hip/hip_runtime.h>
#include <stdint.h>
#include <stdlib.h>
#include <string.h>
#include <string>
#include <vector>
#include "../../include/modsx.h"
#include "kmath.hpp"

namespace mx {

#ifndef MODSX_MAXB
#define MODSX_MAXB 32
#endif
constexpr int MAXB = MODSX_MAXB;
constexpr int PAIR_GROUP = 4;
constexpr int NMS_MAXJ = 1024;
constexpr int MAX_TAPS = 17;

struct BlurJob {
  const float *src;
  float *blur;
  float *resp;
  int rows, cols;
// ... 117 lines not shown
struct Octave {
  int rows, cols;
  float pixelDistance;
  float *blur[8];
  float *resp[8];
};
struct Pyramid {
  int nOct = 0;
  Octave oct[24];
  DevBuf store;
};

void set_error(const std::string &s);
bool gpu_shared();
struct CtxBusy { modsx_ctx *c; explicit CtxBusy(modsx_ctx *c); ~CtxBusy(); CtxBusy(const CtxBusy &) = delete; CtxBusy &operator=(const CtxBusy &) = delete; };
hipError_t ctx_copy(modsx_ctx *c, void *dst, const void *src, size_t bytes, hipMemcpyKind kind);
hipError_t ctx_sync(modsx_ctx *c);
unsigned ctx_mark(modsx_ctx *c);
bool ctx_mark_reached(modsx_ctx *c, unsigned seq);
hipError_t ctx_wait_mark(modsx_ctx *c, unsigned seq);
bool host_wait_runtime();
int host_cpus_per_rank();
#define MX_HIP(expr)                                                                          \
  do {                                                                                        \
    hipError_t e_ = (expr);                                                                   \
    if (e_ != hipSuccess) {                                                                   \
      mx::set_error(std::string(#expr) + ": " + hipGetErrorString(e_));                       \
      return MODSX_ERR_DEVICE;                                                                \
    }                                                                                         \
  } while (0)

std::vector<float> gaussian_kernel(int n, double sigma);
int blur_ksize(float sigma);
void gauss_mask(float *mask, int size);
void circular_gauss_mask(float *mask, int size, float sigma);
const double *atan_lut_host();
inline bool check_borders_host(int w, int h, float ofsx, float ofsy, float a11, float a12, float a21, float a22, int rw, int rh) {
  return check_borders(w, h, ofsx, ofsy, a11, a12, a21, a22, rw, rh);
}
bool invert3(const double *S, double *t);
void rectify(double &a11, double &a12, double &a21, double &a22);

void launch_blur_hess(hipStream_t s, const BlurBatch &b, int nj, int maxRows, int maxCols);
void launch_hessian(hipStream_t s, const BlurBatch &b, int nj, int maxRows, int maxCols);
void launch_resize_half(hipStream_t s, const ResizeBatch &b, int nj, int maxRows, int maxCols);
void launch_nms(hipStream_t s, const NmsBatch &b, const NmsJob *jobs, const int *tilePrefix, const int *tileJob, int nj,
                int nTiles, int4 *queue, unsigned *qcount, unsigned qcap, Candidate *out, unsigned *counter, unsigned cap,
                const int *octFirst = nullptr, int levelsPerOctave = 0);
size_t cand_sort_temp_bytes(unsigned nsort);
int launch_cand_order(hipStream_t s, const Candidate *cand, const unsigned *counter, unsigned nsort, unsigned long long *keys,
                      unsigned long long *keys2, unsigned *idx, unsigned *idx2, void *temp, size_t tempBytes, unsigned long long *tabKey,
                      unsigned *tabRank, unsigned tabSize, unsigned *slotOf, Candidate *out, unsigned *outCount);
constexpr int NMS_QUEUES = 64;
constexpr int NMS_TILE_ROWS = 16;
void launch_gray(hipStream_t s, const void *src, float *dst, size_t n, int channels, int dtype);
struct BaumGeo { int kernel, chunk, nchunks, grid; };
BaumGeo baumberg_geometry(int n, int W, int variant, int chunk, int resident = 0);
int baumberg_resident_waves();
int baumberg_production_variant(int W);
constexpr int BAUM_RANGES = 8, BAUM_COUNTER_STRIDE = 32, BAUM_QUEUE_BYTES = BAUM_RANGES * BAUM_COUNTER_STRIDE * 4;
MX_HD int baum_range_start(int n, int r) { return (int)(((long long)n * r) / BAUM_RANGES); }
bool launch_baumberg(hipStream_t s, const AffJob *jobs, AffOut *out, int n, const float *mask, int W, int maxIter,
                     float convTh, float affInitialSigma, int variant, int chunk, int resident, unsigned *queue, bool queueClean);
constexpr int ATAN_CASES = 2048 + 64;
constexpr int ORI_NV = 1344;
void launch_orientation(hipStream_t s, const OriJob *jobs, float *out, int n, const ImgRef *imgs,
                        const unsigned short *maskIdx, const float *maskW,
                        const unsigned char *binTab, int doHalf, double th, int maxAngles);
void launch_trunc_u8(hipStream_t s, const float *src, uint8_t *dst, size_t n);
size_t mser_sort_blocks(const int *rows, int n);
void launch_mser_sort(hipStream_t s, const uint8_t *const *u8, const int *rows, const int *cols, const size_t *ordOfs, int n, int *blockHist,
                      int *start, int *order);
void launch_expand_blur_tiles(hipStream_t s, const DescJob *jobs, const int *prefixRows, const int *prefixCols, int nJobs,
                              const int *needTab, BlurTile *tilesRows, BlurTile *tilesCols, float2 *rowStarts);
void launch_sample_rows(hipStream_t s, const DescJob *jobs, const BlurTile *tiles, int nTiles, const ImgRef *imgs, const float *taps,
                        const int *needTab, float *dst, const float2 *rowStarts, float *dstGrid);
void launch_blur_cols(hipStream_t s, const BlurTile *tiles, int nTiles, const float *taps, const int *needTab, const float *src,
                      float *dst);
void launch_expand_tiles(hipStream_t s, const int *prefix, int nJobs, int *tileJob);
void launch_patch_sample(hipStream_t s, const DescJob *jobs, const int *tilePrefix, const int *tileJob, int nTiles,
                         const ImgRef *imgs, float *scratch);
void launch_patch_blur(hipStream_t s, const DescJob *jobs, const int *tilePrefix, const int *tileJob, int nTiles,
                       const float *taps, const int *needTab, const float *src, float *dst, int pass);
void launch_describe(hipStream_t s, const DescJob *jobs, int n, const ImgRef *imgs, const float *grid,
                     const int *needTab, const float *coordTab,
                     const float *mask, const unsigned short *maskIdx, int nmask, const float *oTab, const int *bins,
                     const double *wts, int photoNorm, int descTypes, int nOut, double maxBin, const DescOut &outs);
void launch_warp_affine(hipStream_t s, const WarpJob &jb);
void launch_blur_pass(hipStream_t s, const float *src, float *dst, int rows, int cols, const float *taps, int n, int pass, int border = 0);
void launch_sub(hipStream_t s, const float *a, const float *b, float *o, size_t n);
void launch_grad_products(hipStream_t s, const float *img, int rows, int cols, float *xx, float *yy, float *xy);
void launch_harris_combine(hipStream_t s, const float *bxx, const float *byy, const float *bxy, float sigmasq, float *o, size_t n);
void launch_views_warp(hipStream_t s, const ViewJob *jobs, int n, int tiles, int stage);
void launch_views_blur(hipStream_t s, const ViewJob *jobs, int n, int tiles, const float *taps, int pass);
constexpr int VF_TW = 128, VF_TH = 16, VF_RX = 32, VF_RY = 2;
void launch_views_rotblur(hipStream_t s, const ViewJob *jobs, int n, int tiles, const float *taps, int maxRx, int maxRy);
void launch_views_fused(hipStream_t s, const ViewJob *jobs, int n, int tiles, const float *taps, int maxRx, int maxRy);
size_t match_workspace_bytes(int n1, int n2);
void launch_match(hipStream_t s, const uint8_t *d1, int n1, const uint8_t *d2, int n2, const double *pos2,
                  double sqminratio, double contrDistSq, int nn, MatchRow *rows, void *workspace);
#ifndef MODSX_SR_WIN
#define MODSX_SR_WIN 2400
#define MODSX_FC_ROWS 40
#define MODSX_SR_HALF 1
#define MODSX_SR_WGS 8
#endif
#ifndef MODSX_BLUR_LDS_C
#define MODSX_BLUR_LDS_C 9984
#endif
constexpr int MATCH_NN_MAX = 256;
constexpr int MATCH_MAXB = 4;
void launch_match_batch(hipStream_t s, int nb, const uint8_t *const *d1, const int *n1, const uint8_t *const *d2, const int *n2,
                        const double *const *pos2, double sqminratio, double contrDistSq, int nn, MatchRow *const *rows,
                        void *const *workspace, hipEvent_t *evSweep1 = nullptr,
                        const void *const *trainPack = nullptr);
size_t match_train_pack_bytes(int n2);
void launch_match_pack_trains(hipStream_t s, const uint8_t *d2, int n2, const double *pos2, void *pack);
void last_match_geometry(int *qs, int *fat, int *S, int *tilesPerSplit, int *ntilesUB);
struct DbGeo { int TEp, TOp; };
struct DbSet {
  DevBuf store;
  const unsigned char *tiles = nullptr;
  const int *hrow = nullptr;
  DbGeo geo = {0, 0};
  long rows = 0;
  int dev = 0;
};
DbGeo db_geo(long n, long nOdd);
size_t db_tiles_bytes(const DbGeo &g);
size_t db_hrow_bytes(const DbGeo &g);
int db_pack_blocks(long n);
void launch_db_pack(hipStream_t s, const uint8_t *raw, long n, const int2 *base, long nOdd, const DbGeo &geo, unsigned char *tiles,
                    int *hrow);
void launch_db_select(hipStream_t s, int nb, const MatchRow *const *rows, const int *n1, int nn, bool allPoints, int *const *sel, int *cnt,
                      int *const *dmin);
void launch_dbnn_min(hipStream_t s, int nb, const uint8_t *const *d1, const int *n1, int *const *sel, int *cnt, int *const *dmin,
                     const DbSet &db);
struct HammingGeo { int W, WK, tile, ntiles, tilesPerSplit, S, gx; };
HammingGeo hamming_geometry(int n1, int n2, int W, int splits);
size_t hamming_workspace_bytes(const HammingGeo &g, int n1);
void launch_hamming(hipStream_t s, const HammingGeo &g, const uint8_t *d1, int n1, const uint8_t *d2, int n2, int nbytes, void *work,
                    int *nn2, hipEvent_t *ev = nullptr);

}

namespace mx {
#ifdef MODSX_DUP_BUILD
int dup_count(int cls);
#define MX_DUP(cls) for (int dupLeft_ = mx::dup_count(cls); dupLeft_ > 0; dupLeft_--)
#else
#define MX_DUP(cls)
#endif
enum KClass { K_BLUR_HESS = 0, K_HESSIAN, K_RESIZE, K_NMS, K_BAUMBERG, K_ORIENT, K_PATCH_SAMPLE, K_BLUR_ROWS, K_DESCRIBE,
              K_MATCH, K_GRAY, K_WARP, K_VIEW_BLUR, K_BLUR_COLS, K_MATCH_SWEEP1, K_MATCH_DB, K_NCLASS };
struct Profiler {
  bool enabled = false;
  std::vector<hipEvent_t> evA, evB;
  std::vector<int> cls;
  size_t used = 0;
  double ms[K_NCLASS] = {0};
  double work[K_NCLASS] = {0};
  long launches[K_NCLASS] = {0};
};
}

namespace mx {
enum DescCounter { DC_CALLS = 0, DC_CHUNKS, DC_MAX_CHUNKS, DC_CHUNKS_MID_IMAGE, DC_CHUNKS_LATER_IMAGE, DC_JOBS, DC_DIRECT_JOBS,
                   DC_FUSED_WINDOWS, DC_LDS_ROW_TILES, DC_LDS_COL_TILES, DC_SAMPLE_TILES, DC_GLOBAL_ROW_TILES, DC_GLOBAL_COL_TILES,
                   DC_CLAMPED_WINDOWS, DC_N };
}

struct modsx_db { mx::DbSet set; };

struct modsx_image {
  float *d;
  int rows, cols;
  bool owned;
};

struct modsx_ctx {
  int dev;
  hipStream_t stream;
  mx::Pyramid pyr[mx::MAXB];
  mx::DevBuf candSort, candOut;
  size_t lastSurvivors = 0;
  mx::DevBuf nmsJobs, cand, counter, affJobs, affOut, oriJobs, oriOut, descJobs, tilePrefix, taps, imgRefs, scratchA, scratchB,
      descF[mx::MAXB], descU8[mx::MAXB], descAllF[2], descAllU8[2], descAllU8b[2], descCls[2][4][2], descU8x[3][mx::MAXB], shardLocal, pos2, matchRows, matchWork, dbSel, misc, viewTmp[2], viewTaps, viewJobs, viewImg[mx::MAXB], scratchC, needTab, coordTab, tileJob, blurTiles, nmsQueue, rowStarts;
  mx::ImgRef imgRefsHost[mx::MAXB];
  mx::PinBuf hDescB;
  hipEvent_t descEv[2];
  bool descEvPending[2] = {false, false};
  bool descByEvent[2] = {true, true};
  unsigned descMark[2] = {0, 0};
  unsigned *hFlag = nullptr;
  unsigned flagSeq = 0;
  bool waitRuntime = true;
  mx::PinBuf hCand, hAff, hOri, hDesc, hMisc, hNms, hMatch, hViewTaps, hViewJobs, hMser, hRefs;
  float *dSmmMask = nullptr;
  int baumResident = 0;
  int smmW = 0;
  std::vector<uint64_t> candKeys, candKeys2, candClaim;
  std::vector<uint32_t> candOrder, candOrder2;
  float *dOriMask = nullptr;
  unsigned short *dOriIdx = nullptr;
  float *dSiftMask = nullptr;
  unsigned short *dSiftMaskIdx = nullptr;
  int nSiftMask = 0;
  double *dAtan = nullptr;
  unsigned char *dOriBinTab = nullptr;
  float *dSiftOTab = nullptr;
  int *dSiftBins = nullptr;
  double *dSiftW = nullptr;
  double timings[6];
  mx::Profiler prof;
  size_t lastCandCount = 0;
  const mx::DbSet *fginnDb = nullptr;
  long descCnt[mx::DC_N] = {0};
  double hammingMs[2] = {0, 0};
  int busyDepth = 0;
  int shardLane = 0;
  modsx_ctx *peer = nullptr;
  modsx_ctx *half = nullptr;
  mx::DevBuf halfDesc[4];
  void *worker = nullptr;
};
```

mods_amd/csrc/kernels_describe.hip:

```cpp
#include "engine.hpp"
#include "describe_lanes.hpp"

namespace mx {

MX_D int xcd_swizzle(int b, int n) {
  const int G = 8, SG = 8 * G;
  const int full = (n / SG) * SG;
  if (b >= full) return b;
  const int sg = b / SG, r = b - sg * SG;
  const int xcd = r & 7, k = r >> 3;
  return sg * SG + xcd * G + k;
}


__global__ __launch_bounds__(64) void k_expand_tiles(const int *prefix, int nJobs, int *tileJob) {
  const int j = blockIdx.x;
  if (j >= nJobs) return;
  const int b = prefix[j], e = prefix[j + 1];
  for (int t = b + threadIdx.x; t < e; t += 64) tileJob[t] = j;
}

__global__ __launch_bounds__(256) void k_expand_blur_tiles(const DescJob *jobs, const int *prefix0, const int *prefix1, int nJobs,
                                                           const int *needTab, BlurTile *tiles0, BlurTile *tiles1, float2 *rowStart) {
  const int j = blockIdx.x * 256 + threadIdx.x, pass = blockIdx.y;
  if (j >= nJobs) return;
  const int *prefix = pass == 1 ? prefix1 : prefix0;
  const int b = prefix[j], e = prefix[j + 1];
  if (pass == 2) {
    if (b == e) return;
    const DescJob jb = jobs[j];
    float2 *rs = rowStart + jb.scratchOfs;
    const int half = jb.P >> 1;
    float rx = jb.x - (float)half * jb.a12, ry = jb.y - (float)half * jb.a22;
    for (int r = 0; r < jb.P; r++) { rs[r] = make_float2(rx, ry); rx += jb.a12; ry += jb.a22; }
    return;
  }
  if (b == e) return;
  BlurTile *tiles = pass ? tiles1 : tiles0;
  const DescJob jb = jobs[j];
  const int R = jb.ksize >> 1;
  BlurTile bt;
  bt.P = jb.P; bt.NC = jb.NC; bt.n = jb.ksize; bt.tapOfs = jb.tapOfs; bt.needOfs = jb.needOfs;
  bt.job = j; bt.pad = 0;
  { const int NP = (jb.NC + 1) >> 1; bt.magic = ((1 << 20) + NP - 1) / NP; }
  for (int t = b; t < e; t++) {
    if (pass == 0) {
      const int r0 = (t - b) * jb.rows0;
      bt.count = jb.P - r0 < jb.rows0 ? jb.P - r0 : jb.rows0;
      bt.first = r0; bt.lo = 0; bt.span = bt.count;
      bt.srcOfs = jb.scratchOfs + (size_t)r0 * jb.P;
      bt.dstOfs = jb.rowOfs + (size_t)r0 * jb.NC;
    } else {
      const int ro0 = (t - b) * jb.ro1;
      bt.count = jb.NC - ro0 < jb.ro1 ? jb.NC - ro0 : jb.ro1;
      bt.first = ro0;
      bt.lo = needTab[jb.needOfs + ro0] - R;
      bt.span = needTab[jb.needOfs + ro0 + bt.count - 1] + R - bt.lo + 1;
      bt.srcOfs = jb.rowOfs;
      bt.dstOfs = jb.gridOfs + (size_t)ro0 * jb.NC;
    }
    tiles[t] = bt;
  }
}


constexpr int SAMPLE_COLS = 128, SAMPLE_C = 16, SAMPLE_CP = SAMPLE_C + 1, SAMPLE_B = 8;

template <bool TOUCH>
__device__ __forceinline__ void sample_chunk(const ImgRef &im, const float *cx, const float *cy, float *dst, int P, int tot, int nc,
                                             int lane) {
  for (int e0 = lane; e0 < tot; e0 += 64 * SAMPLE_B) {
    float v[SAMPLE_B];
#pragma unroll
    for (int u = 0; u < SAMPLE_B; u++) {
      const int e = e0 + 64 * u, r = e / SAMPLE_C, c = e - r * SAMPLE_C;
      v[u] = (e < tot && c < nc) ? bilinear_tap(as_global(im.d), im.rows, im.cols, cx[r * SAMPLE_CP + c], cy[r * SAMPLE_CP + c], TOUCH) : 0.f;
    }
#pragma unroll
    for (int u = 0; u < SAMPLE_B; u++) {
      const int e = e0 + 64 * u, r = e / SAMPLE_C, c = e - r * SAMPLE_C;
      if (e < tot && c < nc) dst[(size_t)r * P + c] = v[u];
    }
  }
}
// ... 375 lines not shown
  const int n = bt.n, R = n >> 1, RW = P + 2 * R;
#ifdef MODSX_SAMPLE_PAD
  __shared__ volatile char spad_[MODSX_SAMPLE_PAD];
  if (threadIdx.x == 0) spad_[MODSX_SAMPLE_PAD - 1] = 1;
#endif
  __shared__ float win[BLUR_LDS + 2];
  __shared__ int sneed[96];
  __shared__ __attribute__((aligned(16))) float aux[FC_ROWS * FC_LS];
  static_assert(FC_ROWS * FC_LS >= 2 * BLUR_W * SR_WORDS, "aux holds the sampling coordinates");
  float *const cxw = aux + wave_id() * SR_WORDS, *const cyw = aux + (BLUR_W + wave_id()) * SR_WORDS;
  const int nr = bt.count;
  const int lane = threadIdx.x & 63;
  const int wave = __builtin_amdgcn_readfirstlane(threadIdx.x >> 6);
  for (int i = threadIdx.x; i < NC; i += BLUR_T) sneed[i] = needTab[bt.needOfs + i];
  const ImgRef im = imgs[jb.img];
  const float2 *rowStart = rowStarts + jb.scratchOfs;
  sample_rows_tile(bt, jb, im, rowStart, win, cxw, cyw, lane, wave);
  __syncthreads();
  if (R > 0) {
    const int twoR = 2 * R;
    int s = 32 - __clz(twoR - 1);
    s = s > 6 ? 6 : s;
    const int kl = lane & ((1 << s) - 1), rsub = lane >> s, rpp = 64 >> s;
    for (int ri = wave * rpp + rsub; ri < nr; ri += BLUR_W * rpp) {
      float *rowp = win + __umul24((unsigned)ri, (unsigned)RW);
      for (int k = kl; k < twoR; k += 1 << s) {
        if (k < R) rowp[k] = rowp[R];
        else rowp[P + k] = rowp[R + P - 1];
      }
    }
  }
  __syncthreads();
  if (jb.ro1 >= 0) { blur_rows_from_lds(bt, win, sneed, taps, dst + bt.dstOfs, NC); return; }
  blur_rows_from_lds(bt, win, sneed, taps, aux + R * FC_LS, FC_LS);
  __syncthreads();
  for (int i = threadIdx.x; i < R * FC_LS; i += BLUR_T) {
    const int k = i / FC_LS, x = i - k * FC_LS;
    aux[k * FC_LS + x] = aux[R * FC_LS + x];
    aux[(R + P + k) * FC_LS + x] = aux[(R + P - 1) * FC_LS + x];
  }
  __syncthreads();
  blur_cols_from_lds<FC_LS>(NC, n, 0, NC, -R, bt.magic, aux, sneed, taps + bt.tapOfs, dstGrid + jb.gridOfs);
}

template <int LS>
__device__ __forceinline__ void blur_cols_tile(const BlurTile &bt, float *win, int *sneed, const float *__restrict__ taps,
                                               const int *__restrict__ needTab, const float *__restrict__ src,
                                               float *__restrict__ dst) {
  const int P = bt.P, NC = bt.NC;
  const int n = bt.n;
  const int ro0 = bt.first, nro = bt.count, lo = bt.lo, S = bt.span;
  const int lane = threadIdx.x & 63, wave = wave_id();
  for (int i = threadIdx.x; i < NC; i += BLUR_T) sneed[i] = needTab[bt.needOfs + i];
  const float *T = src + bt.srcOfs;
  {
    typedef const float __attribute__((address_space(1))) *gptr;
    typedef float __attribute__((address_space(3))) *lptr;
    for (int si = wave; si < S; si += BLUR_W) {
      int rr = lo + si;
      rr = rr < 0 ? 0 : (rr > P - 1 ? P - 1 : rr);
      const float *a = T + (size_t)rr * NC;
      for (int x0 = 0; x0 < NC; x0 += 64) {
        const int x = x0 + lane;
        if (x < NC) __builtin_amdgcn_global_load_lds((gptr)(a + x), (lptr)(win + si * LS + x0), 4, 0, 0);
      }
    }
    asm volatile("s_waitcnt vmcnt(0)" ::: "memory");
  }
  __syncthreads();
  blur_cols_from_lds<LS>(NC, n, ro0, nro, lo, bt.magic, win, sneed, taps + bt.tapOfs, dst + bt.dstOfs);
}

__global__ __launch_bounds__(BLUR_T) void k_blur_cols_lds(const BlurTile *__restrict__ tiles, const float *__restrict__ taps,
                                                       const int *__restrict__ needTab, const float *__restrict__ src,
                                                       float *__restrict__ dst) {
  const BlurTile bt = tiles[xcd_swizzle(blockIdx.x, gridDim.x)];
  __shared__ __attribute__((aligned(16))) float win[BLUR_LDS_C];
  __shared__ int sneed[96];
  if (bt.NC <= 64) blur_cols_tile<64>(bt, win, sneed, taps, needTab, src, dst);
  else blur_cols_tile<96>(bt, win, sneed, taps, needTab, src, dst);
}

constexpr int PS = 41, NPX = PS * PS;

struct SiftConst {
  int nmask;
};

#ifndef MODSX_DESCRIBE_REGIONS
#define MODSX_DESCRIBE_REGIONS 2
#endif
constexpr int DR = MODSX_DESCRIBE_REGIONS;

__global__ __launch_bounds__(128 * DR) void k_describe(const DescJob *jobs, int n, const ImgRef *imgs, const float *grid,
                                                  const int *needTab, const float *coordTab,
                                                  const float *mask, const unsigned short *maskIdx,
                                                  const float *oTab, const int *binTab, const double *wTab,
                                                  SiftConst sc, int photoNorm, int descTypes, int nOut, double maxBin,
                                                  DescOut outs) {
  const int tidw = threadIdx.x;
  const int reg = __builtin_amdgcn_readfirstlane(tidw >> 7);
  const int tid = tidw & 127;
  const int kreal = blockIdx.x * DR + reg;
  const bool alive = kreal < n;
  const int k = alive ? kreal : n - 1;
  constexpr int NPXP = (NPX + 3) & ~3;
  __shared__ __attribute__((aligned(16))) float buf_[DR][2][NPXP];
  float *const patch = buf_[reg][0], *const bufO = buf_[reg][0];
  constexpr int PER_T = (NPX + 127) / 128;
  float *const bufA = buf_[reg][1];
  __shared__ __attribute__((aligned(16))) double slut_[DR][256];
  __shared__ __attribute__((aligned(16))) unsigned char sbs_[DR][4 * 64];
  __shared__ float4 stab[PS];
  int4 *const smap = reinterpret_cast<int4 *>(bufA);
  float *const sfr = bufA + 168;
  static_assert(PS * 16 <= 168 * 4 && (168 + PS) <= NPXP, "smap (41 x int4) and sfr (41 floats) fit in bufA");
  double *const vec = slut_[reg], *const part = slut_[reg] + 128;
  __shared__ float sstat_[DR][2];
  float *const sstat = sstat_[reg];
  __shared__ double sfac_[DR];
  __shared__ int schanged_[DR];
#ifdef MODSX_DESCRIBE_PAD
  __shared__ volatile char spad_[MODSX_DESCRIBE_PAD];
  if (tidw == 0) spad_[MODSX_DESCRIBE_PAD - 1] = 1;
#endif
  const DescJob jb = jobs[k];
  if (tidw < PS) {
    const float w0 = (float)wTab[tidw], w1 = (float)wTab[PS + tidw];
    const int q = tidw >> 3, b0 = min(max(q - 1, 0), 3), b1 = min(q, 3);
    const float wm = w0 > 0 ? (w1 > 0 ? fminf(w0, w1) : w0) : (w1 > 0 ? w1 : 1.f);
    stab[tidw] = make_float4(w0, w1, wm, __int_as_float(b0 | (b1 << 2)));
  }
  if (jb.P > 0) {
    const float *G = grid + jb.gridOfs;
    const int NC = jb.NC;
    if (tid < PS) {
      const int *mp = needTab + jb.needOfs + NC + 4 * tid;
      const int4 m = make_int4(mp[0], mp[1], mp[2], mp[3]);
      smap[tid] = m;
      sfr[tid] = coordTab[jb.coordOfs + tid] - (float)m.z;
    }
    __syncthreads();
    constexpr int HALF_T = PER_T / 2;
    static_assert(PER_T == 2 * HALF_T, "an even number of samples per thread");
    typedef const char __attribute__((address_space(1))) *gbyte_p;
    const gbyte_p Gb = (gbyte_p)as_global(G);
    const unsigned NCu = (unsigned)NC;
    int rs = tid / PS, cs = tid - rs * PS;
#pragma unroll
    for (int h = 0; h < 2; h++) {
      float g00[HALF_T], g01[HALF_T], g10[HALF_T], g11[HALF_T];
      int rr[HALF_T], cc[HALF_T];
#pragma unroll
      for (int kk = 0; kk < HALF_T; kk++) {
        const int r = rs < PS ? rs : PS - 1, c = rs < PS ? cs : PS - 1;
        rr[kk] = r; cc[kk] = c;
        const int4 mr = smap[r], mc = smap[c];
        const unsigned o0 = __umul24((unsigned)mr.x, NCu), o1 = __umul24((unsigned)mr.y, NCu);
        g00[kk] = *(gcfloat_p)(Gb + ((o0 + (unsigned)mc.x) << 2)); g01[kk] = *(gcfloat_p)(Gb + ((o0 + (unsigned)mc.y) << 2));
        g10[kk] = *(gcfloat_p)(Gb + ((o1 + (unsigned)mc.x) << 2)); g11[kk] = *(gcfloat_p)(Gb + ((o1 + (unsigned)mc.y) << 2));
        cs += 128 - 3 * PS; rs += 3;
        if (cs >= PS) { cs -= PS; rs++; }
      }
      if (h == 0) __syncthreads();
#pragma unroll
      for (int kk = 0; kk < HALF_T; kk++) {
        const int p = tid + 128 * (h * HALF_T + kk);
        if (p < NPX) {
          const int r = rr[kk], c = cc[kk];
          float v = 0.f;
          if (smap[r].w && smap[c].w) {
            const float wx = sfr[c], wyd = sfr[r];
            const float I1 = wx * (g01[kk] - g00[kk]) + g00[kk];
            v = wyd * (wx * (g11[kk] - g10[kk]) + g10[kk] - I1) + I1;
          }
          patch[p] = v;
        }
      }
    }
  } else {
    const ImgRef im = imgs[jb.img];
    const float *src = im.d;
    const int srows = im.rows, scols = im.cols;
    const float ox = jb.x, oy = jb.y, a11 = jb.a11, a12 = jb.a12, a21 = jb.a21, a22 = jb.a22;
    const bool touch = check_borders(scols, srows, ox, oy, a11, a12, a21, a22, PS, PS);
    if (tid < PS) {
      const int half = PS >> 1;
      float rx = ox - (float)half * a12;
      float ry = oy - (float)half * a22;
      for (int j = 0; j < tid; j++) { rx += a12; ry += a22; }
      float WX = rx - (float)half * a11;
      float WY = ry - (float)half * a21;
#pragma unroll 1
      for (int i = 0; i < PS; i++) {
        bufA[tid * PS + i] = WX;
        bufO[tid * PS + i] = WY;
        WX += a11;
        WY += a21;
      }
    }
    __syncthreads();
    float sv[PER_T];
#pragma unroll
    for (int k = 0; k < PER_T; k++) {
      const int p = tid + 128 * k;
      const int r = p / PS, c = p - r * PS;
      sv[k] = p < NPX ? bilinear_tap(as_global(src), srows, scols, bufA[r * PS + c], bufO[r * PS + c], touch) : 0.f;
    }
    __syncthreads();
#pragma unroll
    for (int k = 0; k < PER_T; k++) {
      const int p = tid + 128 * k;
      if (p < NPX) patch[p] = sv[k];
    }
  }
  __syncthreads();
  if (photoNorm) {
    const int nm = sc.nmask, nm4 = (nm + 3) & ~3;
    for (int i = tid; i < nm4; i += 128) bufA[i] = i < nm ? patch[maskIdx[i]] : 0.f;
    __syncthreads();
    if (tidw < DR) {
      float sum = 0.f;
      const float *vals = buf_[tidw][1];
      const float4 *v4 = reinterpret_cast<const float4 *>(vals);
      const int full = nm >> 2;
#pragma unroll 8
      for (int i = 0; i < full; i++) { const float4 v = v4[i]; sum += v.x; sum += v.y; sum += v.z; sum += v.w; }
      for (int i = full * 4; i < nm; i++) sum += vals[i];
      const float gsum = (float)nm;
      sstat_[tidw][0] = sum / gsum;
      sstat_[tidw][1] = gsum;
    }
    __syncthreads();
    const float mean = sstat[0];
    for (int i = tid; i < nm4; i += 128) { const float d = mean - bufA[i]; bufA[i] = i < nm ? d * d : 0.f; }
    __syncthreads();
    if (tidw < DR) {
      float var = 0.f;
      const float *vals = buf_[tidw][1];
      const float4 *v4 = reinterpret_cast<const float4 *>(vals);
      const int full = nm >> 2;
#pragma unroll 8
      for (int i = 0; i < full; i++) { const float4 v = v4[i]; var += v.x; var += v.y; var += v.z; var += v.w; }
      for (int i = full * 4; i < nm; i++) var += vals[i];
      sstat_[tidw][1] = sqrtf(var / sstat_[tidw][1]);
    }
    __syncthreads();
    const float var = sstat[1];
    if (!((double)var < 0.0001)) {
      const float fac = 50.0f / var;
      for (int i = tid; i < NPX; i += 128) {
        float v = 128.f + fac * (patch[i] - mean);
        if (v > 255.f) v = 255.f;
        if (v < 0.f) v = 0.f;
        patch[i] = v;
      }
    }
    __syncthreads();
  }
  float ov[PER_T], vv[PER_T];
#pragma unroll
  for (int k = 0; k < PER_T; k++) {
    const int p = tid + 128 * k;
    ov[k] = 0.f; vv[k] = 0.f;
    if (p >= NPX) continue;
    const int r = p / PS, c = p - r * PS;
    const float xg = patch[c == PS - 1 ? p : p + 1] - patch[c == 0 ? p : p - 1];
    const float yg = patch[r == PS - 1 ? p : p + PS] - patch[r == 0 ? p : p - PS];
    const float g = sqrtf(xg * xg + yg * yg);
    int code, idx;
    const bool special = atan2lut_case(yg, xg, code, idx);
    vv[k] = mask[p] * g;
    ov[k] = oTab[special ? 2048 : code * 256 + idx];
  }
  constexpr int ACS = 145, NAC = 8 * ACS;
  static_assert(NAC * 2 <= 2 * NPXP, "8 skewed copies of 16 x 9 bins fit in bufO + bufA");
  unsigned long long *const acc = reinterpret_cast<unsigned long long *>(buf_[reg][0]);
  __shared__ unsigned smin_[DR][2], smax_[DR][2];
  {
    unsigned mb = 0;
#pragma unroll
    for (int k = 0; k < PER_T; k++) mb = max(mb, __float_as_uint(vv[k]) & 0x7fffffffu);
#pragma unroll
    for (int off = 32; off > 0; off >>= 1) mb = max(mb, (unsigned)__shfl_xor((int)mb, off));
    if ((tid & 63) == 0) smax_[reg][tid >> 6] = mb;
  }
  __syncthreads();
  {
    float4 *const z = reinterpret_cast<float4 *>(buf_[reg][0]);
    for (int i = tid; i < (NAC * 2 + 3) / 4; i += 128) z[i] = make_float4(0.f, 0.f, 0.f, 0.f);
  }
  const unsigned mxb = max(smax_[reg][0], smax_[reg][1]);
  const int E = (int)(mxb >> 23) - 126;
  const bool scalable = mxb >= 0x00800000u && mxb < 0x7f800000u && E >= -60 && E <= 100;
  const float S = __uint_as_float((unsigned)(127 + 47 - (scalable ? E : 47)) << 23);
  __syncthreads();
  unsigned tmin = 0xffffffffu;
  {
    int r = tid / PS, c = tid - r * PS;
#pragma unroll
    for (int k = 0; k < PER_T; k++) {
      const float val = vv[k] * S;
      if (val > 0) {
        const float o = ov[k];
        const int bo0 = (int)o;
        const float wo1 = o - (float)bo0, wo0 = 1.0f - wo1;
        const float4 tr = stab[r], tc = stab[c];
        const int pr = __float_as_int(tr.w), pc = __float_as_int(tc.w);
        const float wc0 = tc.x * val, wc1 = tc.y * val;
        const int ob = (c & 7) * (ACS * 8) + (bo0 & 7) * 8;
        const int r0 = (pr & 3) * 288, r1 = ((pr >> 2) & 3) * 288, c0 = (pc & 3) * 72 + ob, c1 = ((pc >> 2) & 3) * 72 + ob;
        typedef float v2f __attribute__((ext_vector_type(2)));
        const v2f wcv = {wc0, wc1}, wov = {wo0, wo1};
        const v2f va = wcv * tr.x, vb = wcv * tr.y;
        const v2f ts[4] = {wov * va.x, wov * va.y, wov * vb.x, wov * vb.y};
        const int bs[4] = {r0 + c0, r0 + c1, r1 + c0, r1 + c1};
#pragma unroll
        for (int q = 0; q < 4; q++) {
          const double d0 = (double)ts[q].x + 4503599627370496.0, d1 = (double)ts[q].y + 4503599627370496.0;
          unsigned long long *const a = reinterpret_cast<unsigned long long *>(reinterpret_cast<char *>(acc) + bs[q]);
          __hip_atomic_fetch_add(a, (unsigned long long)__double_as_longlong(d0), __ATOMIC_RELAXED, __HIP_MEMORY_SCOPE_WORKGROUP);
          __hip_atomic_fetch_add(a + 1, (unsigned long long)__double_as_longlong(d1), __ATOMIC_RELAXED, __HIP_MEMORY_SCOPE_WORKGROUP);
        }
        const float wom = wo1 > 0 ? fminf(wo0, wo1) : wo0;
        tmin = min(tmin, __float_as_uint((tr.z * (tc.z * val)) * wom) - 1u);
      }
      c += 128 - 3 * PS; r += 3;
      if (c >= PS) { c -= PS; r++; }
    }
  }
#pragma unroll
  for (int off = 32; off > 0; off >>= 1) tmin = min(tmin, (unsigned)__shfl_xor((int)tmin, off));
  if ((tid & 63) == 0) smin_[reg][tid >> 6] = tmin;
  __syncthreads();
  double binT;
  bool inexact;
  {
    const int cell = tid >> 3, slot = tid & 7;
    unsigned long long X = 0;
#pragma unroll
    for (int q = 0; q < 8; q++) {
      constexpr unsigned long long M52 = (1ull << 52) - 1ull;
      X += acc[q * ACS + cell * 9 + slot] & M52;
      if (slot == 0) X += acc[q * ACS + cell * 9 + 8] & M52;
    }
    const unsigned m = min(smin_[reg][0], smin_[reg][1]);
    inexact = !scalable || (m != 0xffffffffu && m + 1u < 0x4b000000u) || (X >> 53) != 0;
    binT = ldexp((double)(unsigned)(X >> 32) * 4294967296.0 + (double)(unsigned)X, (scalable ? E : 47) - 47);
  }
#ifdef MODSX_DESC_ORDERED_ONLY
  inexact = true;
#endif
  const int ordered = __syncthreads_or(inexact);
  if (ordered) {
#pragma unroll
    for (int k = 0; k < PER_T; k++) {
      const int p = tid + 128 * k;
      if (p < NPX) { bufA[p] = vv[k]; bufO[p] = ov[k]; }
    }
    __syncthreads();
  {
    const bool gth = tid < 64;
    const int rb = (tid >> 4) & 3, cb = (tid >> 2) & 3, oa = 2 * (tid & 3), ob = oa + 1, oam = (oa + 7) & 7;
    double accA = 0.0, accB = 0.0;
    float(*const sv0)[64] = reinterpret_cast<float(*)[64]>(vec);
    float(*const sv1)[64] = reinterpret_cast<float(*)[64]>(part);
    unsigned char(*const sbs)[64] = reinterpret_cast<unsigned char(*)[64]>(sbs_[reg]);
#pragma unroll 1
    for (int rr = 0; rr < 16; rr++) {
#pragma unroll
      for (int u = 0; u < 2; u++) {
        const int i = tid + 128 * u, rbi = i >> 6, vc = i & 63;
        const int col = vc < 32 ? vc : vc - 24, r = 8 * rbi + rr;
        const float wrr = rr < 8 ? stab[r].y : stab[r].x;
        const float wcv = (vc < 32 ? stab[col].y : stab[col].x) * bufA[r * PS + col];
        const float v = wrr * wcv;
        const float vcl = v > 0 ? v : 0.f;
        const float o = bufO[r * PS + col];
        const int bo0 = (int)o;
        const float wo1 = o - (float)bo0;
        sv0[rbi][vc] = vcl * (1.0f - wo1);
        sv1[rbi][vc] = vcl * wo1;
        sbs[rbi][vc] = (unsigned char)(bo0 & 7);
      }
      __syncthreads();
      if (gth) {
#pragma unroll
        for (int seg = 0; seg < 4; seg++) {
          const int sx = (seg < 2 ? 0 : 24) + 8 * cb + 4 * seg;
          const float4 p0v = *reinterpret_cast<const float4 *>(&sv0[rb][sx]);
          const float4 p1v = *reinterpret_cast<const float4 *>(&sv1[rb][sx]);
          const unsigned b4 = *reinterpret_cast<const unsigned *>(&sbs[rb][sx]);
          const float p0s[4] = {p0v.x, p0v.y, p0v.z, p0v.w};
          const float p1s[4] = {p1v.x, p1v.y, p1v.z, p1v.w};
#pragma unroll
          for (int e = 0; e < 4; e++) {
            const int b0 = (int)((b4 >> (8 * e)) & 0xff);
            const bool isA = b0 == oa, isAm = b0 == oam, isB = b0 == ob;
            const float ta = isA ? p0s[e] : (isAm ? p1s[e] : 0.f);
            const float tb = isB ? p0s[e] : (isA ? p1s[e] : 0.f);
            accA += (double)ta;
            accB += (double)tb;
          }
        }
      }
      __syncthreads();
    }
    if (gth) { vec[(rb * 4 + cb) * 8 + oa] = accA; vec[(rb * 4 + cb) * 8 + ob] = accB; }
  }
  } else vec[tid] = binT;
  __syncthreads();
  const double rawBin = vec[tid];
#pragma unroll 1
  for (int ot = 0; ot < nOut; ot++) {
  const int descType = (descTypes >> (4 * ot)) & 15;
  if (ot) {
    __syncthreads();
    vec[tid] = rawBin;
    __syncthreads();
  }
  const bool rootsift = (descType & 1) != 0;
  if (descType >= 2) {
    const int sb = tid >> 2, j = tid & 3;
    const double h = tid < 64 ? vec[sb * 8 + j] + vec[sb * 8 + j + 4] : 0.0;
    __syncthreads();
    vec[tid] = h;
    __syncthreads();
  }
  bool active = true;
  for (int pass = 0; pass < 2; pass++) {
    if (tid < 32 && active) {
      const double s0 = vec[4 * tid] * vec[4 * tid], s1 = vec[4 * tid + 1] * vec[4 * tid + 1],
                   s2 = vec[4 * tid + 2] * vec[4 * tid + 2], s3 = vec[4 * tid + 3] * vec[4 * tid + 3];
      part[tid] = s0 + s1 + s2 + s3;
    }
    __syncthreads();
    if (tid == 0 && active) {
      double len = 0.0;
#pragma unroll
      for (int i = 0; i < 32; i++) len += part[i];
      len = sqrt(len);
      sfac_[reg] = 1.0 / len;
      schanged_[reg] = 0;
    }
    __syncthreads();
    if (active) vec[tid] *= sfac_[reg];
    __syncthreads();
    if (pass == 0) {
      if (vec[tid] > maxBin) { vec[tid] = maxBin; schanged_[reg] = 1; }
      __syncthreads();
      if (!schanged_[reg]) active = false;
    }
  }
  __syncthreads();
  if (rootsift) {
    if (tidw < DR) {
      const double *vq = slut_[tidw];
      double sum = 0.;
#pragma unroll 16
      for (int i = 0; i < 128; i++) sum += fabs(vq[i]);
      sfac_[tidw] = sum;
    }
    __syncthreads();
    vec[tid] = sqrt(vec[tid] / sfac_[reg]);
  }
  {
    int b;
    if (rootsift) b = (int)(512.0 * vec[tid] + 0.5);
    else b = (int)((double)512.0f * vec[tid] + 0.5);
    b = b < 255 ? b : 255;
    b = b > 0 ? b : 0;
    if (alive) {
      if (ot == 0) {
        outs.f[jb.img][(size_t)jb.outIdx * 128 + tid] = (float)b;
        outs.u8[jb.img][(size_t)jb.outIdx * 128 + tid] = (uint8_t)b;
      } else
        outs.u8x[ot - 1][jb.img][(size_t)jb.outIdx * 128 + tid] = (uint8_t)b;
    }
  }
  }
}

void launch_expand_tiles(hipStream_t s, const int *prefix, int nJobs, int *tileJob) {
  if (nJobs <= 0) return;
  hipLaunchKernelGGL(k_expand_tiles, dim3(nJobs), dim3(64), 0, s, prefix, nJobs, tileJob);
}
void launch_patch_sample(hipStream_t s, const DescJob *jobs, const int *tilePrefix, const int *tileJob, int nTiles,
                         const ImgRef *imgs, float *scratch) {
  if (nTiles <= 0) return;
  hipLaunchKernelGGL(k_patch_sample, dim3(8 * ((nTiles + 7) / 8)), dim3(64), 0, s, jobs, tilePrefix, tileJob, imgs, scratch, nTiles);
}
void launch_expand_blur_tiles(hipStream_t s, const DescJob *jobs, const int *prefixRows, const int *prefixCols, int nJobs,
                              const int *needTab, BlurTile *tilesRows, BlurTile *tilesCols, float2 *rowStarts) {
  if (nJobs > 0) MX_DUP(K_PATCH_SAMPLE) hipLaunchKernelGGL(k_expand_blur_tiles, dim3((nJobs + 255) / 256, 3), dim3(256), 0, s, jobs, prefixRows, prefixCols, nJobs, needTab,
                                    tilesRows, tilesCols, rowStarts);
}
void launch_sample_rows(hipStream_t s, const DescJob *jobs, const BlurTile *tiles, int nTiles, const ImgRef *imgs, const float *taps,
                        const int *needTab, float *dst, const float2 *rowStarts, float *dstGrid) {
  if (nTiles <= 0) return;
  MX_DUP(K_BLUR_ROWS) hipLaunchKernelGGL(k_sample_rows_lds, dim3(8 * ((nTiles + 7) / 8)), dim3(BLUR_T), 0, s, tiles, jobs, imgs, taps, needTab, dst, nTiles,
                     rowStarts, dstGrid);
}
void launch_blur_cols(hipStream_t s, const BlurTile *tiles, int nTiles, const float *taps, const int *needTab, const float *src,
                      float *dst) {
  if (nTiles > 0) MX_DUP(K_BLUR_COLS) hipLaunchKernelGGL(k_blur_cols_lds, dim3(nTiles), dim3(BLUR_T), 0, s, tiles, taps, needTab, src, dst);
}
void launch_patch_blur(hipStream_t s, const DescJob *jobs, const int *tilePrefix, const int *tileJob, int nTiles,
                       const float *taps, const int *needTab, const float *src, float *dst, int pass) {
  if (nTiles <= 0) return;
  hipLaunchKernelGGL(k_patch_blur, dim3(nTiles), dim3(256), 0, s, jobs, tilePrefix, tileJob, taps, needTab, src, dst, pass);
}
void launch_describe(hipStream_t s, const DescJob *jobs, int n, const ImgRef *imgs, const float *grid,
                     const int *needTab, const float *coordTab, const float *mask, const unsigned short *maskIdx, int nmask, const float *oTab, const int *bins,
                     const double *wts, int photoNorm, int descTypes, int nOut, double maxBin, const DescOut &outs) {
  if (n <= 0) return;
  SiftConst sc;
  sc.nmask = nmask;
  MX_DUP(K_DESCRIBE) hipLaunchKernelGGL(k_describe, dim3((n + DR - 1) / DR), dim3(128 * DR), 0, s, jobs, n, imgs, grid, needTab, coordTab, mask, maskIdx, oTab, bins,
                     wts, sc,
                     photoNorm, descTypes, nOut, maxBin, outs);
}

}
```

Before: 236.0.

## Iterate SIFT gradient pass over a precomputed disc pixel list instead of raster

Adds a host-built list of the pixels inside the circular Gaussian mask, packed with row and column, and a templated describe kernel that walks this list (10 entries per thread) instead of all 41x41 pixels (14 per thread). The aim is to cut the gradient, atan-LUT and binning work spent on zero-weight corner pixels, and to drop the per-step raster index arithmetic. In exchange the ordered fallback must zero the shared buffers before scattering, and the list path keeps packed coordinates in registers. The scalable exponent bound is also tightened, which sends more patches to the ordered path. An env var turns the path off, and debug entry points are added.

```diff
diff --git a/include/modsx.h b/include/modsx.h
--- a/include/modsx.h
+++ b/include/modsx.h
@@ -224,6 +224,9 @@
 int modsx_debug_check_borders(const float *tuples, int n, unsigned char *touch);
 int modsx_debug_describe_lanes(int P, long *counts);
 int modsx_debug_describe_lane_map(int rows, int nc, int *rule, int *map, int cap);
+int modsx_debug_describe_disc(int *counts, unsigned *list, int cap_list, unsigned *read_set, int cap_read, float *mask);
+int modsx_debug_describe_classes(modsx_ctx *ctx, const modsx_image *img, const modsx_region *regs, int n, double mrSize,
+                                 int photoNorm, const int *types, int ntypes, double maxBinValue, float *desc, unsigned char *u8);
 int modsx_last_timings(modsx_ctx *ctx, double *ms6);
 
 int modsx_set_vs_pars(const double *scale_set, int ns, const double *tilt_set, int nt, double phi_base,
diff --git a/mods_amd/__init__.py b/mods_amd/__init__.py
--- a/mods_amd/__init__.py
+++ b/mods_amd/__init__.py
@@ -101,6 +101,7 @@
            "modsx_debug_orientation_counts", "modsx_debug_reproject_certain_drop", "modsx_debug_describe_plan",
            "modsx_debug_baumberg_geometry", "modsx_debug_baumberg_geometry_ctx", "modsx_debug_baumberg_variant",
            "modsx_debug_baumberg", "modsx_debug_check_borders", "modsx_debug_describe_lanes", "modsx_debug_describe_lane_map",
+           "modsx_debug_describe_disc", "modsx_debug_describe_classes",
            "modsx_rep_create", "modsx_rep_free", "modsx_rep_add_views", "modsx_rep_append", "modsx_rep_class",
            "modsx_rep_match_fginn", "modsx_match_reps", "modsx_match_one_to_many",
            "modsx_match_hamming", "modsx_match_hamming_device", "modsx_hamming_tentatives", "modsx_debug_match_hamming",
@@ -181,6 +182,9 @@
         L.modsx_debug_check_borders.argtypes = [C.c_void_p, C.c_int, C.c_void_p]
         L.modsx_debug_describe_lanes.argtypes = [C.c_int, C.c_void_p]
         L.modsx_debug_describe_lane_map.argtypes = [C.c_int, C.c_int, C.c_void_p, C.c_void_p, C.c_int]
+        L.modsx_debug_describe_disc.argtypes = [C.c_void_p, C.c_void_p, C.c_int, C.c_void_p, C.c_int, C.c_void_p]
+        L.modsx_debug_describe_classes.argtypes = [C.c_void_p, C.c_void_p, C.c_void_p, C.c_int, C.c_double, C.c_int, C.c_void_p, C.c_int,
+                                                   C.c_double, C.c_void_p, C.c_void_p]
         L.modsx_rep_create.restype = C.c_void_p
         L.modsx_rep_create.argtypes = [C.c_void_p]
         L.modsx_rep_free.restype = None
@@ -627,6 +631,15 @@
                "describe_regions")
         return desc
 
+    def describe_classes(self, img, regs, types=(1,), mr_size=5.1962, photo_norm=1, max_bin=0.2):
+        regs = np.ascontiguousarray(regs, REGION)
+        t = np.ascontiguousarray(types, np.int32)
+        desc = np.zeros((len(regs), 128), np.float32)
+        u8 = np.zeros((len(t), len(regs), 128), np.uint8)
+        _check(lib().modsx_debug_describe_classes(self._c(), C.c_void_p(img.h), _p(regs), len(regs), C.c_double(mr_size), photo_norm,
+                                                  _p(t), len(t), C.c_double(max_bin), _p(desc), _p(u8)), "describe_classes")
+        return desc, u8
+
     def describe_counters(self):
         v = (C.c_long * len(DESCRIBE_COUNTERS))()
         n = _check(lib().modsx_describe_counters(self._c(), v, len(DESCRIBE_COUNTERS)), "describe_counters")
@@ -976,6 +989,24 @@
     return out
 
 
+DESCRIBE_DISC_COUNTS = ("nmask", "list_entries", "nread", "read_entries", "per_thread", "slots_needed",
+                        "raster_grad_issued", "raster_gather_issued", "raster_holding",
+                        "list_grad_issued", "list_gather_issued", "list_holding", "list_form")
+
+
+def describe_disc():
+    k = np.zeros(len(DESCRIBE_DISC_COUNTS), np.int32)
+    _check(lib().modsx_debug_describe_disc(_p(k), None, 0, None, 0, None), "describe_disc")
+    out = dict(zip(DESCRIBE_DISC_COUNTS, (int(x) for x in k)))
+    dl, rs = np.zeros(out["list_entries"], np.uint32), np.zeros(out["read_entries"], np.uint32)
+    mask = np.zeros((41, 41), np.float32)
+    _check(lib().modsx_debug_describe_disc(_p(k), _p(dl), len(dl), _p(rs), len(rs), _p(mask)), "describe_disc")
+    for name, w in (("list", dl), ("read_set", rs)):
+        out[name] = np.stack([w & 2047, (w >> 11) & 63, (w >> 17) & 63, (w >> 23) & 1], axis=1).astype(np.int32)
+    out["mask"] = mask
+    return out
+
+
 def orientation_counts(reset=False):
     a, b = C.c_ulonglong(), C.c_ulonglong()
     lib().modsx_debug_orientation_counts(C.byref(a), C.byref(b), int(reset))
diff --git a/mods_amd/csrc/capi.hip b/mods_amd/csrc/capi.hip
--- a/mods_amd/csrc/capi.hip
+++ b/mods_amd/csrc/capi.hip
@@ -10,6 +10,7 @@
 #include "engine_api.hpp"
 #include "describe_plan.hpp"
 #include "describe_lanes.hpp"
+#include "describe_disc.hpp"
 
 using namespace mx;
 
@@ -410,6 +411,26 @@
   return tot;
 }
 
+int modsx_debug_describe_disc(int *counts, unsigned *list, int cap_list, unsigned *read_set, int cap_read, float *mask) {
+  NEED(counts);
+  if (cap_list < 0 || (cap_list > 0 && !list) || cap_read < 0 || (cap_read > 0 && !read_set)) {
+    mx::set_error("modsx_debug_describe_disc: bad argument"); return MODSX_ERR_ARG;
+  }
+  std::vector<float> m(mx::DISC_NPX);
+  mx::circular_gauss_mask(m.data(), mx::DISC_PS, 0);
+  int nmask = 0, nread = 0;
+  const std::vector<unsigned> dl = mx::disc_list(m.data(), nmask), rs = mx::disc_read_set(m.data(), nread);
+  const mx::DiscSlots a = mx::disc_slots_raster(m.data()), b = mx::disc_slots_list(dl);
+  const int v[13] = {nmask, (int)dl.size(), nread, (int)rs.size(), mx::DISC_PER_M, (nmask + 63) / 64,
+                     a.gradIssued, a.gatherIssued, a.holding, b.gradIssued, b.gatherIssued, b.holding,
+                     mx::describe_list_form() && nmask <= mx::DISC_CAP ? 1 : 0};
+  for (int q = 0; q < 13; q++) counts[q] = v[q];
+  for (int i = 0; i < cap_list && i < (int)dl.size(); i++) list[i] = dl[i];
+  for (int i = 0; i < cap_read && i < (int)rs.size(); i++) read_set[i] = rs[i];
+  if (mask) for (int i = 0; i < mx::DISC_NPX; i++) mask[i] = m[i];
+  return MODSX_OK;
+}
+
 int modsx_debug_baumberg(modsx_ctx *ctx, const modsx_image *const *planes, int nplanes, const int *plane_of, const float *xyspd,
                          int n, const modsx_hessaff_params *par, int variant, int chunk, float *u, int *ok, int *iters,
                          int *geometry, int *handed_out) {
@@ -490,6 +511,34 @@
   int rc = describe_batch(ctx, imgs, 1, v, mrSize, patchSize, fast_extraction, photoNorm, desc_type, maxBinValue, hosts,
                           nullptr, nullptr);
   if (rc) return rc;
+  return n;
+}
+
+int modsx_debug_describe_classes(modsx_ctx *ctx, const modsx_image *img, const modsx_region *regs, int n, double mrSize,
+                                 int photoNorm, const int *types, int ntypes, double maxBinValue, float *desc, unsigned char *u8) {
+  NEED(ctx); NEED(img); NEED(types);
+  if (n < 0 || (n > 0 && (!regs || !desc || !u8)) || ntypes < 1 || ntypes > MODSX_MAX_DESC) {
+    mx::set_error("modsx_debug_describe_classes: bad argument"); return MODSX_ERR_ARG;
+  }
+  mx::DescSet ds;
+  ds.n = ntypes;
+  for (int k = 0; k < ntypes; k++) {
+    if (types[k] < MODSX_DESC_SIFT || types[k] > MODSX_DESC_HALF_ROOT_SIFT) { mx::set_error("descriptor type"); return MODSX_ERR_ARG; }
+    ds.type[k] = types[k];
+  }
+  hipSetDevice(ctx->dev);
+  std::vector<modsx_region> v[1];
+  v[0].assign(regs, regs + n);
+  const modsx_image *imgs[1] = {img};
+  float *hosts[1] = {desc};
+  const int rc = describe_batch(ctx, imgs, 1, v, mrSize, 41, 0, photoNorm, ds.type[0], maxBinValue, hosts, nullptr, nullptr, &ds);
+  if (rc) return rc;
+  for (int k = 0; k < ntypes && n > 0; k++) {
+    const void *src = k == 0 ? ctx->descU8[0].p : ctx->descU8x[k - 1][0].p;
+    if (hipMemcpy(u8 + (size_t)k * n * 128, src, (size_t)n * 128, hipMemcpyDeviceToHost) != hipSuccess) {
+      mx::set_error("modsx_debug_describe_classes: copy failed"); return MODSX_ERR_DEVICE;
+    }
+  }
   return n;
 }
 
diff --git a/mods_amd/csrc/describe_disc.hpp b/mods_amd/csrc/describe_disc.hpp
--- /dev/null
+++ b/mods_amd/csrc/describe_disc.hpp
@@ -0,0 +1,74 @@
+#pragma once
+#include <vector>
+#include "kmath.hpp"
+
+namespace mx {
+
+constexpr int DISC_PS = 41, DISC_NPX = DISC_PS * DISC_PS;
+constexpr int DISC_T = 128;
+constexpr int DISC_PER_M = 10;
+constexpr int DISC_CAP = DISC_T * DISC_PER_M;
+constexpr int DISC_PER_T = (DISC_NPX + DISC_T - 1) / DISC_T;
+
+constexpr unsigned DISC_PAD = 1u << 23;
+constexpr unsigned disc_entry(int r, int c) { return (unsigned)(r * DISC_PS + c) | (unsigned)r << 11 | (unsigned)c << 17; }
+MX_HD int disc_p(unsigned w) { return (int)(w & 2047u); }
+MX_HD int disc_r(unsigned w) { return (int)((w >> 11) & 63u); }
+MX_HD int disc_c(unsigned w) { return (int)((w >> 17) & 63u); }
+MX_HD bool disc_is_pad(unsigned w) { return (w & DISC_PAD) != 0; }
+MX_HD unsigned disc_half(unsigned w) { return (w >> 11) & 0x1fffu; }
+MX_HD int disc_half_r(unsigned h) { return (int)(h & 63u); }
+MX_HD int disc_half_c(unsigned h) { return (int)((h >> 6) & 63u); }
+MX_HD bool disc_half_is_pad(unsigned h) { return (h & 0x1000u) != 0; }
+
+inline std::vector<unsigned> disc_list(const float *mask, int &nmask) {
+  std::vector<unsigned> v;
+  for (int r = 0; r < DISC_PS; r++)
+    for (int c = 0; c < DISC_PS; c++)
+      if (mask[r * DISC_PS + c] > 0) v.push_back(disc_entry(r, c));
+  nmask = (int)v.size();
+  while (v.size() % DISC_T || v.size() < (size_t)DISC_CAP) v.push_back(disc_entry(DISC_PS / 2, DISC_PS / 2) | DISC_PAD);
+  return v;
+}
+
+inline std::vector<unsigned> disc_read_set(const float *mask, int &nread) {
+  std::vector<unsigned char> in(DISC_NPX, 0);
+  for (int r = 0; r < DISC_PS; r++)
+    for (int c = 0; c < DISC_PS; c++) {
+      if (!(mask[r * DISC_PS + c] > 0)) continue;
+      in[r * DISC_PS + c] = 1;
+      if (r > 0) in[(r - 1) * DISC_PS + c] = 1;
+      if (r < DISC_PS - 1) in[(r + 1) * DISC_PS + c] = 1;
+      if (c > 0) in[r * DISC_PS + c - 1] = 1;
+      if (c < DISC_PS - 1) in[r * DISC_PS + c + 1] = 1;
+    }
+  std::vector<unsigned> v;
+  for (int p = 0; p < DISC_NPX; p++) if (in[p]) v.push_back(disc_entry(p / DISC_PS, p % DISC_PS));
+  nread = (int)v.size();
+  while (v.size() % DISC_T || v.size() < (size_t)DISC_CAP) v.push_back(disc_entry(DISC_PS / 2, DISC_PS / 2) | DISC_PAD);
+  return v;
+}
+
+struct DiscSlots { int gradIssued, gatherIssued, holding; };
+inline DiscSlots disc_slots_raster(const float *mask) {
+  DiscSlots s = {2 * DISC_PER_T, 0, 0};
+  for (int s0 = 0; s0 < DISC_T * DISC_PER_T; s0 += 64) {
+    bool any = false;
+    for (int p = s0; p < s0 + 64 && p < DISC_NPX; p++) any = any || mask[p] > 0;
+    s.holding += any;
+  }
+  s.gatherIssued = s.holding;
+  return s;
+}
+inline DiscSlots disc_slots_list(const std::vector<unsigned> &list) {
+  DiscSlots s = {2 * DISC_PER_M, 0, 0};
+  for (size_t s0 = 0; s0 < (size_t)DISC_CAP; s0 += 64) {
+    bool any = false;
+    for (size_t e = s0; e < s0 + 64 && e < list.size(); e++) any = any || !disc_is_pad(list[e]);
+    s.holding += any;
+  }
+  s.gatherIssued = s.holding;
+  return s;
+}
+
+}
diff --git a/mods_amd/csrc/engine.hip b/mods_amd/csrc/engine.hip
--- a/mods_amd/csrc/engine.hip
+++ b/mods_amd/csrc/engine.hip
@@ -9,6 +9,7 @@
 #include <string>
 #include "engine_api.hpp"
 #include "describe_plan.hpp"
+#include "describe_disc.hpp"
 
 #ifdef MODSX_DUP_BUILD
 namespace mx {
@@ -245,6 +246,11 @@
     c->nSiftMask = (int)idx.size();
     MX_HIP(hipMalloc(&c->dSiftMaskIdx, idx.size() * 2));
     MX_HIP(hipMemcpy(c->dSiftMaskIdx, idx.data(), idx.size() * 2, hipMemcpyHostToDevice));
+    int nd = 0;
+    const std::vector<unsigned> disc = disc_list(m.data(), nd);
+    if (nd != c->nSiftMask) { set_error("descriptor mask: the two pixel lists differ"); return MODSX_ERR_ARG; }
+    MX_HIP(hipMalloc(&c->dSiftDisc, disc.size() * 4));
+    MX_HIP(hipMemcpy(c->dSiftDisc, disc.data(), disc.size() * 4, hipMemcpyHostToDevice));
   }
   MX_HIP(hipMalloc(&c->dAtan, 256 * 8));
   MX_HIP(hipMemcpy(c->dAtan, atan_lut_host(), 256 * 8, hipMemcpyHostToDevice));
@@ -341,7 +347,7 @@
   c->candSort.release(); c->candOut.release();
   PinBuf *pins[] = {&c->hCand, &c->hAff, &c->hOri, &c->hDesc, &c->hMisc, &c->hNms, &c->hMatch, &c->hViewTaps, &c->hViewJobs, &c->hMser};
   for (PinBuf *b : pins) b->release();
-  hipFree(c->dSmmMask); hipFree(c->dOriMask); hipFree(c->dOriIdx); hipFree(c->dSiftMask); hipFree(c->dSiftMaskIdx); hipFree(c->dAtan); hipFree(c->dOriBinTab); hipFree(c->dSiftOTab); hipFree(c->dSiftBins);
+  hipFree(c->dSmmMask); hipFree(c->dOriMask); hipFree(c->dOriIdx); hipFree(c->dSiftMask); hipFree(c->dSiftMaskIdx); hipFree(c->dSiftDisc); hipFree(c->dAtan); hipFree(c->dOriBinTab); hipFree(c->dSiftOTab); hipFree(c->dSiftBins);
   hipFree(c->dSiftW);
   for (int i = 0; i < 2; i++) hipEventDestroy(c->descEv[i]);
   c->hDescB.release(); c->hRefs.release();
@@ -620,7 +626,7 @@
                       (float *)c->scratchC.p, 1); }
   ProfScope psd(c, K_DESCRIBE, (double)nj * 128 * ds.n);
   launch_describe(s, dj, (int)nj, (ImgRef *)c->imgRefs.p, (float *)c->scratchC.p, dNeed, dCoord,
-                  c->dSiftMask, c->dSiftMaskIdx, c->nSiftMask, c->dSiftOTab,
+                  c->dSiftMask, c->dSiftMaskIdx, c->nSiftMask, c->dSiftDisc, c->dSiftOTab,
                   c->dSiftBins, c->dSiftW, photoNorm, ds.packed(), ds.n, maxBin, outs);
   return MODSX_OK;
 }
diff --git a/mods_amd/csrc/engine.hpp b/mods_amd/csrc/engine.hpp
--- a/mods_amd/csrc/engine.hpp
+++ b/mods_amd/csrc/engine.hpp
@@ -223,10 +223,11 @@
                          const ImgRef *imgs, float *scratch);
 void launch_patch_blur(hipStream_t s, const DescJob *jobs, const int *tilePrefix, const int *tileJob, int nTiles,
                        const float *taps, const int *needTab, const float *src, float *dst, int pass);
+bool describe_list_form();
 void launch_describe(hipStream_t s, const DescJob *jobs, int n, const ImgRef *imgs, const float *grid,
                      const int *needTab, const float *coordTab,
-                     const float *mask, const unsigned short *maskIdx, int nmask, const float *oTab, const int *bins,
-                     const double *wts, int photoNorm, int descTypes, int nOut, double maxBin, const DescOut &outs);
+                     const float *mask, const unsigned short *maskIdx, int nmask, const unsigned *discTab, const float *oTab,
+                     const int *bins, const double *wts, int photoNorm, int descTypes, int nOut, double maxBin, const DescOut &outs);
 void launch_warp_affine(hipStream_t s, const WarpJob &jb);
 void launch_blur_pass(hipStream_t s, const float *src, float *dst, int rows, int cols, const float *taps, int n, int pass, int border = 0);
 void launch_sub(hipStream_t s, const float *a, const float *b, float *o, size_t n);
@@ -347,6 +348,7 @@
   float *dSiftMask = nullptr;
   unsigned short *dSiftMaskIdx = nullptr;
   int nSiftMask = 0;
+  unsigned *dSiftDisc = nullptr;
   double *dAtan = nullptr;
   unsigned char *dOriBinTab = nullptr;
   float *dSiftOTab = nullptr;
diff --git a/mods_amd/csrc/kernels_describe.hip b/mods_amd/csrc/kernels_describe.hip
--- a/mods_amd/csrc/kernels_describe.hip
+++ b/mods_amd/csrc/kernels_describe.hip
@@ -1,5 +1,6 @@
 #include "engine.hpp"
 #include "describe_lanes.hpp"
+#include "describe_disc.hpp"
 
 namespace mx {
 
@@ -541,6 +542,7 @@
 }
 
 constexpr int PS = 41, NPX = PS * PS;
+static_assert(PS == DISC_PS && NPX == DISC_NPX, "describe_disc.hpp describes this patch");
 
 struct SiftConst {
   int nmask;
@@ -551,9 +553,10 @@
 #endif
 constexpr int DR = MODSX_DESCRIBE_REGIONS;
 
+template <bool DISC>
 __global__ __launch_bounds__(128 * DR) void k_describe(const DescJob *jobs, int n, const ImgRef *imgs, const float *grid,
                                                   const int *needTab, const float *coordTab,
-                                                  const float *mask, const unsigned short *maskIdx,
+                                                  const float *mask, const unsigned short *maskIdx, const unsigned *discTab,
                                                   const float *oTab, const int *binTab, const double *wTab,
                                                   SiftConst sc, int photoNorm, int descTypes, int nOut, double maxBin,
                                                   DescOut outs) {
@@ -567,6 +570,8 @@
   __shared__ __attribute__((aligned(16))) float buf_[DR][2][NPXP];
   float *const patch = buf_[reg][0], *const bufO = buf_[reg][0];
   constexpr int PER_T = (NPX + 127) / 128;
+  static_assert(PER_T == DISC_PER_T && DISC_T == 128, "describe_disc.hpp describes these passes");
+  constexpr int PER_G = DISC ? DISC_PER_M : PER_T;
   float *const bufA = buf_[reg][1];
   __shared__ __attribute__((aligned(16))) double slut_[DR][256];
   __shared__ __attribute__((aligned(16))) unsigned char sbs_[DR][4 * 64];
@@ -717,13 +722,23 @@
     }
     __syncthreads();
   }
-  float ov[PER_T], vv[PER_T];
-#pragma unroll
-  for (int k = 0; k < PER_T; k++) {
-    const int p = tid + 128 * k;
+  float ov[PER_G], vv[PER_G];
+  static_assert(PER_G % 2 == 0, "two entries per word of pk");
+  unsigned pk[PER_G / 2];
+#pragma unroll
+  for (int k = 0; k < PER_G; k++) {
+    int p, r, c;
+    bool pad = false;
     ov[k] = 0.f; vv[k] = 0.f;
-    if (p >= NPX) continue;
-    const int r = p / PS, c = p - r * PS;
+    if (DISC) {
+      const unsigned w = discTab[tid + 128 * k];
+      p = disc_p(w); r = disc_r(w); c = disc_c(w); pad = disc_is_pad(w);
+      pk[k >> 1] = (k & 1) ? pk[k >> 1] | disc_half(w) << 16 : disc_half(w);
+    } else {
+      p = tid + 128 * k;
+      if (p >= NPX) continue;
+      r = p / PS; c = p - r * PS;
+    }
     const float xg = patch[c == PS - 1 ? p : p + 1] - patch[c == 0 ? p : p - 1];
     const float yg = patch[r == PS - 1 ? p : p + PS] - patch[r == 0 ? p : p - PS];
     const float g = sqrtf(xg * xg + yg * yg);
@@ -731,6 +746,7 @@
     const bool special = atan2lut_case(yg, xg, code, idx);
     vv[k] = mask[p] * g;
     ov[k] = oTab[special ? 2048 : code * 256 + idx];
+    if (DISC && pad) { vv[k] = 0.f; ov[k] = 0.f; }
   }
   constexpr int ACS = 145, NAC = 8 * ACS;
   static_assert(NAC * 2 <= 2 * NPXP, "8 skewed copies of 16 x 9 bins fit in bufO + bufA");
@@ -739,7 +755,7 @@
   {
     unsigned mb = 0;
 #pragma unroll
-    for (int k = 0; k < PER_T; k++) mb = max(mb, __float_as_uint(vv[k]) & 0x7fffffffu);
+    for (int k = 0; k < PER_G; k++) mb = max(mb, __float_as_uint(vv[k]) & 0x7fffffffu);
 #pragma unroll
     for (int off = 32; off > 0; off >>= 1) mb = max(mb, (unsigned)__shfl_xor((int)mb, off));
     if ((tid & 63) == 0) smax_[reg][tid >> 6] = mb;
@@ -751,14 +767,19 @@
   }
   const unsigned mxb = max(smax_[reg][0], smax_[reg][1]);
   const int E = (int)(mxb >> 23) - 126;
-  const bool scalable = mxb >= 0x00800000u && mxb < 0x7f800000u && E >= -60 && E <= 100;
+  const bool scalable = mxb >= 0x00800000u && mxb < 0x7f800000u && E >= -60 && E <= 47;
   const float S = __uint_as_float((unsigned)(127 + 47 - (scalable ? E : 47)) << 23);
   __syncthreads();
   unsigned tmin = 0xffffffffu;
   {
     int r = tid / PS, c = tid - r * PS;
 #pragma unroll
-    for (int k = 0; k < PER_T; k++) {
+    for (int k = 0; k < PER_G; k++) {
+      if (DISC) {
+        if (!(k & 1)) asm volatile("" : "+v"(pk[k >> 1]));
+        const unsigned h = pk[k >> 1] >> (16 * (k & 1));
+        r = disc_half_r(h); c = disc_half_c(h);
+      }
       const float val = vv[k] * S;
       if (val > 0) {
         const float o = ov[k];
@@ -784,8 +805,10 @@
         const float wom = wo1 > 0 ? fminf(wo0, wo1) : wo0;
         tmin = min(tmin, __float_as_uint((tr.z * (tc.z * val)) * wom) - 1u);
       }
-      c += 128 - 3 * PS; r += 3;
-      if (c >= PS) { c -= PS; r++; }
+      if (!DISC) {
+        c += 128 - 3 * PS; r += 3;
+        if (c >= PS) { c -= PS; r++; }
+      }
     }
   }
 #pragma unroll
@@ -812,10 +835,22 @@
 #endif
   const int ordered = __syncthreads_or(inexact);
   if (ordered) {
-#pragma unroll
-    for (int k = 0; k < PER_T; k++) {
-      const int p = tid + 128 * k;
-      if (p < NPX) { bufA[p] = vv[k]; bufO[p] = ov[k]; }
+    if (DISC) {
+      float4 *const z = reinterpret_cast<float4 *>(buf_[reg][0]);
+      for (int i = tid; i < 2 * NPXP / 4; i += 128) z[i] = make_float4(0.f, 0.f, 0.f, 0.f);
+      __syncthreads();
+#pragma unroll
+      for (int k = 0; k < PER_G; k++) {
+        const unsigned h = pk[k >> 1] >> (16 * (k & 1));
+        const int p = disc_half_r(h) * PS + disc_half_c(h);
+        if (!disc_half_is_pad(h)) { bufA[p] = vv[k]; bufO[p] = ov[k]; }
+      }
+    } else {
+#pragma unroll
+      for (int k = 0; k < PER_G; k++) {
+        const int p = tid + 128 * k;
+        if (p < NPX) { bufA[p] = vv[k]; bufO[p] = ov[k]; }
+      }
     }
     __syncthreads();
   {
@@ -969,15 +1004,24 @@
   if (nTiles <= 0) return;
   hipLaunchKernelGGL(k_patch_blur, dim3(nTiles), dim3(256), 0, s, jobs, tilePrefix, tileJob, taps, needTab, src, dst, pass);
 }
+bool describe_list_form() {
+  static const bool on = !(getenv("MODSX_DESCRIBE_DISC") && atoi(getenv("MODSX_DESCRIBE_DISC")) == 0);
+  return on;
+}
 void launch_describe(hipStream_t s, const DescJob *jobs, int n, const ImgRef *imgs, const float *grid,
-                     const int *needTab, const float *coordTab, const float *mask, const unsigned short *maskIdx, int nmask, const float *oTab, const int *bins,
+                     const int *needTab, const float *coordTab, const float *mask, const unsigned short *maskIdx, int nmask,
+                     const unsigned *discTab, const float *oTab, const int *bins,
                      const double *wts, int photoNorm, int descTypes, int nOut, double maxBin, const DescOut &outs) {
   if (n <= 0) return;
   SiftConst sc;
   sc.nmask = nmask;
-  MX_DUP(K_DESCRIBE) hipLaunchKernelGGL(k_describe, dim3((n + DR - 1) / DR), dim3(128 * DR), 0, s, jobs, n, imgs, grid, needTab, coordTab, mask, maskIdx, oTab, bins,
-                     wts, sc,
-                     photoNorm, descTypes, nOut, maxBin, outs);
-}
-
-}
+  const dim3 g((n + DR - 1) / DR), b(128 * DR);
+  if (describe_list_form() && discTab && nmask <= DISC_CAP)
+    MX_DUP(K_DESCRIBE) hipLaunchKernelGGL(k_describe<true>, g, b, 0, s, jobs, n, imgs, grid, needTab, coordTab, mask, maskIdx, discTab, oTab,
+                                          bins, wts, sc, photoNorm, descTypes, nOut, maxBin, outs);
+  else
+    MX_DUP(K_DESCRIBE) hipLaunchKernelGGL(k_describe<false>, g, b, 0, s, jobs, n, imgs, grid, needTab, coordTab, mask, maskIdx, discTab, oTab,
+                                          bins, wts, sc, photoNorm, descTypes, nOut, maxBin, outs);
+}
+
+}
```

Result: no change. 236.7 (median of 5 runs) (+0.3%).
